# alvinwan/neural-backed-decision-trees

Measured on AMD Instinct MI355X. Metric: images/sec training SoftNBDT WRN28x10 CIFAR10, higher is better.
Workload: dtype bf16; 1 GPU; WideResNet-28-10 + SoftTreeSupLoss (induced-wrn28_10_cifar10, 10 leaves), CIFAR10-shaped 3x32x32, SGD m=0.9 wd=5e-4; batch_per_gpu=512, global_batch=512, parallelism=dp1

## Files before the change

include/nbdt_hip.h:

```cpp
#ifndef NBDT_HIP_H
#define NBDT_HIP_H

#include <stdint.h>

#ifdef __cplusplus
extern "C" {
#endif

#define NBDT_OK 0
#define NBDT_EINVAL (-1)
#define NBDT_EHIP (-2)
#define NBDT_ENOMEM (-3)

#define NBDT_F32 0
#define NBDT_BF16 1
#define NBDT_F16 2

const char* nbdt_last_error(void);
const char* nbdt_debug_last_igemm(void);
const char* nbdt_debug_last_igemm_full(void);
const char* nbdt_debug_last_wgrad(void);
int nbdt_version(void);
int nbdt_set_deterministic(int32_t on);
int nbdt_get_deterministic(void);
int nbdt_set_wgrad_store_epilogue(int32_t on);
int nbdt_get_wgrad_store_epilogue(void);
int nbdt_set_reserved_cus(int32_t n);
int nbdt_get_reserved_cus(void);
int nbdt_device_count(void);

int nbdt_weight_tile_batched(const void* src_bf16, const int64_t* table, int32_t n, int64_t total_tiles,
                             void* dst_bf16, void* stream);

typedef struct nbdt_tree nbdt_tree;
int nbdt_tree_create(int device, int num_classes, int num_inodes, int root,
                     const int32_t* node_off, const int32_t* slot_off, const int32_t* slot_cls,
                     const int32_t* cls_off, const int32_t* cls_slot, const int32_t* slot_next,
                     nbdt_tree** out);
int nbdt_tree_destroy(nbdt_tree* t);
int nbdt_tree_max_depth(const nbdt_tree* t);


int nbdt_soft_forward(const nbdt_tree* t, const void* z, int ztype, int64_t B, int64_t ldz,
                      float* P, void* stream);
int nbdt_soft_backward(const nbdt_tree* t, const void* z, int ztype, int64_t B, int64_t ldz,
                       const float* gP, float* gz, void* stream);
int nbdt_soft_tree_loss(const nbdt_tree* t, const void* z, int ztype, int64_t B, int64_t ldz,
                        const int64_t* y, float w_xent, float w_tree, float grad_scale,
                        float* row_loss, float* loss, float* gz, void* stream);
int nbdt_head_soft_tree_loss(const nbdt_tree* t, const float* pooled, const float* W, const float* bias, int64_t B,
                             int32_t K, const int64_t* y, float w_xent, float w_tree, float grad_scale,
                             float* row_loss, float* loss, float* z_out, float* gpooled, float* gW, float* gb,
                             void* stream);

int nbdt_hard_tree_loss(const nbdt_tree* t, const void* z, int ztype, int64_t B, int64_t ldz,
                        const int64_t* y, float w_xent, float w_node, float grad_scale,
                        float* row_loss, float* loss, float* gz, void* stream);
int nbdt_node_logits_backward(const nbdt_tree* t, const float* gs, int64_t B, float* gz, void* stream);
int nbdt_hard_forward(const nbdt_tree* t, const void* z, int ztype, int64_t B, int64_t ldz,
                      int64_t* pred, float* onehot, int32_t* path_node, int32_t* path_child,
                      float* path_prob, float* path_entropy, void* stream);
int nbdt_node_outputs(const nbdt_tree* t, const void* z, int ztype, int64_t B, int64_t ldz,
                      float* logits, float* probs, int64_t* preds, float* entropy, void* stream);

typedef struct nbdt_conv_desc {
  int32_t B, gh, gw;
  int32_t cin, cout;
  int32_t ntaps;
  int32_t tap_off[9];
  int32_t w_tap[9];
  int32_t w_ntaps;
  int32_t in_bs, in_hs, in_ws, in_base;
  int32_t out_bs, out_hs, out_ws, out_base;
  int32_t accumulate;
  int32_t wide_tile;
  int32_t ksplit;
  uint64_t w_tiled;
} nbdt_conv_desc;
int nbdt_conv_plan(const nbdt_conv_desc* d, int32_t* form, int32_t* ksplit);
int nbdt_conv_igemm(const nbdt_conv_desc* d, const void* in, const void* w, void* out,
                    const void* residual, void* stream);

int nbdt_conv_igemm_multi(const nbdt_conv_desc* descs, int32_t n, const void* in, const void* w, void* out,
                          void* stream);

typedef struct nbdt_conv_seg_slice {
  int32_t tensor;
  int32_t ch0;
  int32_t ntaps;
  int32_t tap[9];
  int32_t w_matrix;
  int32_t w_off[9];
} nbdt_conv_seg_slice;
typedef struct nbdt_conv_seg_class {
  int32_t nslices;
  const nbdt_conv_seg_slice* slices;
  int32_t out_bs, out_hs, out_ws, out_base;
} nbdt_conv_seg_class;
#define NBDT_SEG_MAX_SLICES 64
typedef struct nbdt_conv_seg_desc {
  int32_t B, gh, gw;
  int32_t cout;
  int32_t ntensors;
  int32_t pix_stride[4];
  int32_t nmatrices;
  int32_t w_row_stride[4];
  int32_t nclasses;
  nbdt_conv_seg_class cls[4];
  int32_t tile;
  int32_t nbuf;
} nbdt_conv_seg_desc;
int nbdt_conv_seg_create(const nbdt_conv_seg_desc* d, void** plan);
int nbdt_conv_seg_destroy(void* plan);
int nbdt_conv_seg_info(void* plan, int32_t* tile, int32_t* nbuf, int32_t* steps, int32_t* max_rounds,
                       int64_t* w_tile_elems);
int nbdt_conv_seg_tile_weights(void* plan, const void* const* w, void* w_tiles, void* stream);
int nbdt_conv_seg(void* plan, const void* const* in, const void* w_tiles, void* out, const void* residual,
                  float* bn_partials, void* stream);
int nbdt_conv_seg_steps(void* plan, int32_t cls, int32_t* out8, int32_t max_steps, int32_t* npro);

int nbdt_conv_igemm_stats(const nbdt_conv_desc* d, const void* in, const void* w, void* out,
                          const void* residual, float* bn_partials, void* stream);

int nbdt_conv_igemm_bnbwd(const nbdt_conv_desc* d, const void* in, const void* w, void* out,
                          const void* bn_x, const float* save_mean, const float* save_rstd,
                          const float* gamma, const float* beta, float* bn_partials, void* stream);
int nbdt_conv_igemm_affine(const nbdt_conv_desc* d, const void* in, const void* w, void* out,
                           const void* residual, const float* scale, const float* shift, int32_t act,
                           void* stream);

typedef struct nbdt_wgrad_desc {
  int32_t B, gh, gw;
  int32_t cin, cout;
  int32_t ntaps;
  int32_t tap_off[9];
  int32_t w_tap[9];
  int32_t w_ntaps;
  int32_t x_bs, x_hs, x_ws, x_base;
  int32_t g_bs, g_hs, g_ws, g_base;
  int32_t variant;
  int32_t cu_budget;
} nbdt_wgrad_desc;
int nbdt_conv_wgrad(const nbdt_wgrad_desc* d, const void* x, const void* gy, float* dw,
                    void* stream);
int nbdt_conv_wgrad_blocks(const nbdt_wgrad_desc* d);

int nbdt_weight_prep(const float* w, int32_t cout, int32_t taps, int32_t cin, void* w_bf16,
                     void* wd_bf16, void* stream);

int nbdt_weight_prep_batched(const float* flat, const int64_t* table, int32_t n_layers, int64_t total_tiles,
                             void* wd_flat, void* stream);

#define NBDT_BN_SLOTS 32
int nbdt_bn_stats(const void* x, int32_t B, int32_t H, int32_t W, int32_t C, float eps,
                  float momentum, float* running_mean, float* running_var, float* scratch,
                  float* save_mean, float* save_rstd, void* stream);
int nbdt_bn_finalize(int32_t B, int32_t H, int32_t W, int32_t C, float eps, float momentum,
                     float* running_mean, float* running_var, const float* bn_partials, float* save_mean,
                     float* save_rstd, void* stream);
int nbdt_bn_apply(const void* x, const float* save_mean, const float* save_rstd, const float* gamma,
                  const float* beta, const void* residual, int32_t relu, int32_t B, int32_t H,
                  int32_t W, int32_t C, void* y, void* stream);
int nbdt_bn_apply_s2d(const void* x, const float* save_mean, const float* save_rstd, const float* gamma,
                      const float* beta, int32_t relu, int32_t B, int32_t H, int32_t W, int32_t C, void* y,
                      void* stream);
int nbdt_bn_bwd_reduce(const void* gy, const void* y, const void* x, const float* save_mean,
                       const float* save_rstd, const float* gamma, const float* beta, int32_t relu,
                       int32_t B, int32_t H, int32_t W, int32_t C, float* scratch, float* dsum,
                       float* dgamma, float* dbeta, void* stream);
int nbdt_bn_bwd_fold(int32_t B, int32_t H, int32_t W, int32_t C, const float* bn_partials, float* dsum,
                     float* dgamma, float* dbeta, void* stream);
int nbdt_bn_bwd_apply(const void* gy, const void* y, const void* x, const float* save_mean,
                      const float* save_rstd, const float* gamma, const float* beta, const float* dsum,
                      const void* gx_add, int32_t relu, int32_t B, int32_t H, int32_t W, int32_t C,
                      void* gx, void* g_resid, void* stream);
int nbdt_bn_bwd_apply_cus(const void* gy, const void* x, const float* save_mean, const float* save_rstd,
                          const float* gamma, const float* beta, const float* dsum, const void* gx_add,
                          int32_t B, int32_t H, int32_t W, int32_t C, void* gx, int32_t cus, void* stream);
int nbdt_bn_bwd_reduce_cus(const void* gy, const void* x, const float* save_mean, const float* save_rstd,
                           const float* gamma, const float* beta, int32_t B, int32_t H, int32_t W, int32_t C,
                           float* scratch, float* dsum, float* dgamma, float* dbeta, int32_t cus, void* stream);
int nbdt_bn_bwd_cus(const void* gy, const void* x, const float* save_mean, const float* save_rstd, const float* gamma,
                    const float* beta, const void* gx_add, int32_t B, int32_t H, int32_t W, int32_t C, float* slots,
                    float* slots_other, float* dsum, float* dgamma, float* dbeta, void* gx, int32_t cus,
                    void* stream);
int nbdt_bn_relu_pool(const void* x, const float* save_mean, const float* save_rstd,
                      const float* gamma, const float* beta, int32_t B, int32_t H, int32_t W,
                      int32_t C, float* pooled, void* stream);
int nbdt_pool_bn_bwd_reduce(const float* gpooled, const void* x, const float* save_mean,
                            const float* save_rstd, const float* gamma, const float* beta,
                            int32_t B, int32_t H, int32_t W, int32_t C, float* scratch, float* dsum,
                            float* dgamma, float* dbeta, void* stream);
int nbdt_pool_bn_bwd_apply(const float* gpooled, const void* x, const float* save_mean,
                           const float* save_rstd, const float* gamma, const float* beta,
                           const float* dsum, int32_t B, int32_t H, int32_t W, int32_t C, void* gx,
                           void* stream);

#define NBDT_ACT_NONE 0
#define NBDT_ACT_RELU 1
#define NBDT_ACT_SWISH 2
int nbdt_bn_act_apply(const void* x, const float* save_mean, const float* save_rstd, const float* gamma,
                      const float* beta, int32_t act, const float* gate, const void* residual, int32_t B,
                      int32_t H, int32_t W, int32_t C, void* y, void* stream);
int nbdt_bn_act_pool(const void* x, const float* save_mean, const float* save_rstd, const float* gamma,
                     const float* beta, int32_t act, const void* mul, float scale, int32_t B, int32_t H,
                     int32_t W, int32_t C, float* out, void* stream);
int nbdt_bn_act_bwd(const void* gu, const float* gate, const float* gpool, const void* x,
                    const float* save_mean, const float* save_rstd, const float* gamma, const float* beta,
                    int32_t act, const void* gx_add, int32_t B, int32_t H, int32_t W, int32_t C,
                    float* scratch, float* dsum, float* dgamma, float* dbeta, void* gx, void* stream);
int nbdt_dwconv_fwd(const void* x, const float* w, int32_t B, int32_t H, int32_t W, int32_t C, int32_t k,
                    int32_t stride, void* y, float* bn_scratch , void* stream);
int nbdt_dwconv_bwd_data(const void* gy, const float* w, int32_t B, int32_t H, int32_t W, int32_t C,
                         int32_t k, int32_t stride, void* gx, void* stream);
int nbdt_dwconv_bwd_data_bn(const void* gy, const float* w, int32_t B, int32_t H, int32_t W, int32_t C, int32_t k,
                            void* gx, const void* bn_x, const float* save_mean, const float* save_rstd,
                            const float* gamma, const float* beta, float* scratch, void* stream);
int nbdt_bn_act_bwd_apply(const void* gu, const void* x, const float* save_mean, const float* save_rstd,
                          const float* gamma, const float* beta, int32_t act, const void* gx_add, int32_t B, int32_t H,
                          int32_t W, int32_t C, float* scratch, float* dsum, float* dgamma, float* dbeta, void* gx,
                          void* stream);
int nbdt_bn_act_se_sums(const void* gu, const void* x, const float* save_mean, const float* save_rstd,
                        const float* gamma, const float* beta, int32_t act, int32_t B, int32_t H, int32_t W, int32_t C,
                        float* sums, void* stream);
int nbdt_bn_act_se_bwd_apply(const void* gu, const float* gate, const float* gpool, float* sums, const void* x,
                             const float* save_mean, const float* save_rstd, const float* gamma, const float* beta,
                             int32_t act, int32_t B, int32_t H, int32_t W, int32_t C, float* dsum, float* dgamma,
                             float* dbeta, void* gx, void* stream);
int nbdt_dwconv_bwd_weight(const void* x, const void* gy, int32_t B, int32_t H, int32_t W, int32_t C,
                           int32_t k, int32_t stride, float* dw, void* stream);
int nbdt_se_gate_fwd(const float* pooled, const float* w1, const float* b1, const float* w2,
                     const float* b2, int32_t B, int32_t C, int32_t C_real, int32_t S, float* pre1,
                     float* gate, void* stream);
int nbdt_se_gate_bwd(const float* dgate, const float* gate, const float* pre1, const float* pooled,
                     const float* w1, const float* w2, int32_t B, int32_t C, int32_t C_real, int32_t S,
                     float* dpre2, float* dpre1, float* gpool, float* dw1, float* db1, float* dw2,
                     float* db2, void* stream);
int nbdt_se_param_grad(const float* dpre2, const float* dpre1, const float* pre1, const float* pooled,
                       int32_t B, int32_t C, int32_t C_real, int32_t S, float* dw1, float* db1, float* dw2,
                       float* db2, void* stream);
int nbdt_dropout_fwd(const float* x, int64_t n, float p, uint32_t seed, uint8_t* mask, float* y,
                     void* stream);
int nbdt_dropout_bwd(const float* gy, int64_t n, float p, const uint8_t* mask, float* gx, void* stream);

int nbdt_ref_conv(const nbdt_conv_desc* d, const float* in, const float* w, float* out, const float* residual,
                  void* stream);
int nbdt_ref_wgrad(const nbdt_wgrad_desc* d, const float* x, const float* gy, float* dw, void* stream);
int nbdt_ref_conv_seg(void* plan, const float* const* in, const float* const* w, float* out, const float* residual,
                      void* stream);
int nbdt_ref_bn_stats(const float* x, int32_t B, int32_t H, int32_t W, int32_t C, float eps, float momentum,
                      float* running_mean, float* running_var, float* save_mean, float* save_rstd, float* partials,
                      void* stream);
int nbdt_ref_bn_apply(const float* x, const float* save_mean, const float* save_rstd, const float* gamma,
                      const float* beta, const float* residual, int32_t relu, int32_t B, int32_t H, int32_t W,
                      int32_t C, float* y, void* stream);
int nbdt_ref_bn_apply_s2d(const float* x, const float* save_mean, const float* save_rstd, const float* gamma,
                          const float* beta, int32_t relu, int32_t B, int32_t H, int32_t W, int32_t C, float* y,
                          void* stream);
int nbdt_ref_bn_bwd(const float* gy, const float* gpooled, const float* y, const float* x, const float* save_mean,
                    const float* save_rstd, const float* gamma, const float* beta, int32_t relu, const float* gx_add,
                    int32_t B, int32_t H, int32_t W, int32_t C, int32_t reduce, float* dsum, float* dgamma,
                    float* dbeta, float* gx, float* g_resid, void* stream);
int nbdt_ref_bn_relu_pool(const float* x, const float* save_mean, const float* save_rstd, const float* gamma,
                          const float* beta, int32_t B, int32_t H, int32_t W, int32_t C, float* pooled, void* stream);
int nbdt_ref_stem_conv(const float* img, const float* w, int32_t B, int32_t H, int32_t W, int32_t cout_real,
                       int32_t cpad, int32_t stride, float* out, void* stream);
int nbdt_ref_stem_wgrad(const float* img, const float* gy, int32_t B, int32_t H, int32_t W, int32_t cout_real,
                        int32_t cpad, int32_t stride, float* dw, void* stream);
int nbdt_ref_bn_act_apply(const float* x, const float* save_mean, const float* save_rstd, const float* gamma,
                          const float* beta, int32_t act, const float* gate, const float* residual, int32_t B, int32_t H,
                          int32_t W, int32_t C, float* y, void* stream);
int nbdt_ref_bn_act_pool(const float* x, const float* save_mean, const float* save_rstd, const float* gamma,
                         const float* beta, int32_t act, const float* mul, float scale, int32_t B, int32_t H, int32_t W,
                         int32_t C, float* out, void* stream);
int nbdt_ref_bn_act_bwd(const float* gu, const float* gate, const float* gpool, const float* x, const float* save_mean,
                        const float* save_rstd, const float* gamma, const float* beta, int32_t act, const float* gx_add,
                        int32_t B, int32_t H, int32_t W, int32_t C, float* dsum, float* dgamma, float* dbeta, float* gx,
                        void* stream);
int nbdt_ref_dwconv_fwd(const float* x, const float* w, int32_t B, int32_t H, int32_t W, int32_t C, int32_t k,
                        int32_t stride, float* y, void* stream);
int nbdt_ref_dwconv_bwd_data(const float* gy, const float* w, int32_t B, int32_t H, int32_t W, int32_t C, int32_t k,
                             int32_t stride, float* gx, void* stream);
int nbdt_ref_dwconv_bwd_weight(const float* x, const float* gy, int32_t B, int32_t H, int32_t W, int32_t C, int32_t k,
                               int32_t stride, float* dw, void* stream);

int nbdt_stem_conv(const float* img, const float* w, int32_t B, int32_t H, int32_t W,
                   int32_t cout_real, int32_t cpad, int32_t stride, void* out, void* stream);
int nbdt_stem_wgrad(const float* img, const void* gy, int32_t B, int32_t H, int32_t W,
                    int32_t cout_real, int32_t cpad, int32_t stride, float* dw, void* stream);
int nbdt_linear_fwd(const float* x, const float* w, const float* b, int32_t B, int32_t K, int32_t N,
                    float* z, void* stream);
int nbdt_linear_bwd(const float* x, const float* w, const float* gz, int32_t B, int32_t K, int32_t N,
                    float* gx, float* gw, float* gb, void* stream);
int nbdt_sgd_step(float* p, float* g, float* buf, int64_t n, float lr, float momentum,
                  float weight_decay, float grad_scale, void* p_bf16, int32_t zero_grad, void* stream);

int nbdt_probe_mfma_stream(int32_t blocks, int32_t iters, float* sink, void* stream);
int nbdt_probe_lds_mfma(int32_t blocks, int32_t iters, int32_t variant, float* sink, void* stream);
// ... 6 lines not shown
```

neural-backed-decision-trees_amd/csrc/common.h:

```cpp
#pragma once
#include <hip/hip_runtime.h>
#include <hip/hip_bf16.h>
#include <hip/hip_fp16.h>
#include <stdint.h>
#include <stdio.h>
#include <string.h>

#include <mutex>

#include "../../include/nbdt_hip.h"

#if !defined(NBDT_TIMING_BUILD) &&                                                                                    \
    (defined(NBDT_WPP_NO_EPI) || defined(NBDT_WKS_NO_EXCHANGE) || defined(NBDT_WKS_DMA_IN_M) || defined(NBDT_WPP_MIN_STAGES) || defined(NBDT_WPP_FRAC8) || defined(NBDT_PP_KFRAC5) ||    \
     defined(NBDT_DMA_WTILED_FAKE) || defined(NBDT_PP_DUMMY_VALU) || defined(NBDT_PP_NO_PERSIST) || defined(NBDT_PP_NO_PAD) ||                    \
     defined(NBDT_HALO_NO_ACCUMULATE) || defined(NBDT_DW_TARGET) || defined(NBDT_DW_U) || defined(NBDT_HEAD_SPB) ||    \
     defined(NBDT_EPI_TIMING) || defined(NBDT_EPI_STATS_ATOMICS) || defined(NBDT_WGT_NSTAGE) || defined(NBDT_NO_XCD_CONTIGUOUS) || defined(NBDT_CUS_IN_FLIGHT) || defined(NBDT_NT_MIN_MB) || defined(NBDT_PLAIN_STORES) ||                      \
     (defined(NBDT_HEAD_SKIP) && (NBDT_HEAD_SKIP + 0) != 0) || (defined(NBDT_PP_ABLATE) && (NBDT_PP_ABLATE + 0) != 0) || \
     (defined(NBDT_PP_SCHED) && (NBDT_PP_SCHED + 0) != 0) || (defined(NBDT_PP_TIMING) && (NBDT_PP_TIMING + 0) != 0) ||  \
     (defined(NBDT_WPP_TIMING) && (NBDT_WPP_TIMING + 0) != 0) || (defined(NBDT_SEG_TIMING) && (NBDT_SEG_TIMING + 0) != 0) || (defined(NBDT_RULES_TIMING) && (NBDT_RULES_TIMING + 0) != 0))
#error "timing-experiment switch without -DNBDT_TIMING_BUILD: these switches change what the kernels compute (csrc/common.h)"
#endif
#ifdef NBDT_TIMING_BUILD
extern "C" __attribute__((weak, used, visibility("default"))) int nbdt_timing_build() { return 1; }
#endif

namespace nbdt {

extern thread_local char g_err[512];

inline int fail(int code, const char* fmt, const char* a = "", const char* b = "") {
  snprintf(g_err, sizeof(g_err), fmt, a, b);
  return code;
}

#define NBDT_HIP_CHECK(expr)                                                              \
  do {                                                                                    \
    hipError_t _e = (expr);                                                               \
    if (_e != hipSuccess) return nbdt::fail(NBDT_EHIP, "%s: %s", #expr, hipGetErrorString(_e)); \
  } while (0)

#define NBDT_REQUIRE(cond, msg)                                       \
  do {                                                                \
    if (!(cond)) return nbdt::fail(NBDT_EINVAL, "%s (%s)", msg, #cond); \
  } while (0)

#define NBDT_LAUNCH_CHECK() NBDT_HIP_CHECK(hipGetLastError())

struct DeviceAttr {
  static constexpr int kMaxDevices = 64;
  std::mutex m;
  size_t bytes[kMaxDevices] = {};
  int dev = 0;
  bool need(size_t want) {
    int d = 0;
    (void)hipGetDevice(&d);
    if (d < 0 || d >= kMaxDevices) d = kMaxDevices - 1;
    m.lock();
    dev = d;
    if (bytes[d] >= want && want > 0) { m.unlock(); return false; }
    return true;
  }
  void done(size_t want) { bytes[dev] = want ? want : 1; m.unlock(); }
  void abort() { m.unlock(); }
};
#define NBDT_ATTR_CHECK(site, expr)                                                       \
  do {                                                                                    \
    hipError_t _e = (expr);                                                               \
    if (_e != hipSuccess) { (site).abort(); return nbdt::fail(NBDT_EHIP, "%s: %s", #expr, hipGetErrorString(_e)); } \
  } while (0)

bool deterministic();
bool wgrad_store_epilogue();
int reserved_cus();
float* det_rows(hipStream_t st, size_t floats);
const char* det_rows_why();
int det_fold(hipStream_t st, const float* rows, int nrows, size_t n, float* dst);

typedef unsigned short bf16_t;

__device__ __forceinline__ float bf16_to_f32(bf16_t v) {
  return __uint_as_float(((unsigned)v) << 16);
}
__device__ __forceinline__ bf16_t f32_to_bf16(float f) {
  unsigned u = __float_as_uint(f);
  if ((u & 0x7fffffffu) > 0x7f800000u) return (bf16_t)((u >> 16) | 0x40);
  u += 0x7fffu + ((u >> 16) & 1u);
  return (bf16_t)(u >> 16);
}
__device__ __forceinline__ unsigned pack_bf16x2(float lo, float hi) {
  unsigned r;
  asm("v_cvt_pk_bf16_f32 %0, %1, %2" : "=v"(r) : "v"(lo), "v"(hi));
  return r;
}

struct FastDiv {
  unsigned mul, sh, d;
};
inline FastDiv make_fastdiv(unsigned d) {
  FastDiv f;
  f.d = d;
  if (d == 1) { f.mul = 0; f.sh = 0; return f; }
  unsigned s = 0;
  while ((1ull << s) < d) ++s;
  const unsigned long long num = 1ull << (31 + s);
  f.mul = (unsigned)((num + d - 1) / d);
  f.sh = s - 1;
  return f;
}
__device__ __forceinline__ unsigned fdiv(unsigned n, const FastDiv& f) {
  return f.d == 1 ? n : (__umulhi(n, f.mul) >> f.sh);
}

struct PadGeom {
  int B, H, W, C;
  int npix;
  int row;
  int img;
  FastDiv div_w, div_h;
};
inline PadGeom make_geom(int B, int H, int W, int C) {
  PadGeom g;
  g.B = B; g.H = H; g.W = W; g.C = C;
  g.npix = B * H * W;
  g.row = (W + 2) * C;
  g.img = (H + 2) * g.row;
  g.div_w = make_fastdiv((unsigned)W);
  g.div_h = make_fastdiv((unsigned)H);
  return g;
}
__device__ __forceinline__ int pad_offset(const PadGeom& g, int p) {
  const unsigned t = fdiv((unsigned)p, g.div_w);
  const int w = p - (int)t * g.W;
  const unsigned b = fdiv(t, g.div_h);
  const int h = (int)t - (int)b * g.H;
  return (int)b * g.img + (h + 1) * g.row + (w + 1) * g.C;
}

int wgrad_dma(const nbdt_wgrad_desc* d, const void* x, const void* gy, float* dw, hipStream_t st);

bool wgrad_taps_applicable(const nbdt_wgrad_desc* d);
int wgrad_taps(const nbdt_wgrad_desc* d, const void* x, const void* gy, float* dw, hipStream_t st);
int wgrad_taps_blocks(const nbdt_wgrad_desc* d);

bool wgrad_s2d_applicable(const nbdt_wgrad_desc* d);
int wgrad_s2d(const nbdt_wgrad_desc* d, const void* x, const void* gy, float* dw, hipStream_t st);
int wgrad_s2d_blocks(const nbdt_wgrad_desc* d);

struct BnBwdArgs {
  const void* x;
  const float *mean, *rstd, *gamma, *beta;
  const float *aff_scale = nullptr, *aff_shift = nullptr;
  int aff_act = 0;
};
int conv_igemm_dma(const nbdt_conv_desc* d, const void* in, const void* w, void* out, const void* res,
                   float* stats, const BnBwdArgs* bn, int M, hipStream_t st);
int conv_igemm_dma_multi(const nbdt_conv_desc* descs, int n, const void* in, const void* w, void* out, hipStream_t st);

struct HaloGeom {
  int ib, rb;
  int hw2;
  int himg;
  int hp;
  int a_instr;
  int a_bytes;
  int blocks_per_img;
  int nwv;
  int mw;
  int lpitch, limg;
  int pad, dv;
  int row_magic;
};
bool conv_halo_applicable(const nbdt_conv_desc* d, int M, HaloGeom* hg);
int conv_ksplit_rule(const nbdt_conv_desc& d, int nt, int items);
int conv_halo_items(const nbdt_conv_desc& d, const HaloGeom& hg, int M, int* nt_out);
extern thread_local const char* g_last_wgrad;
extern thread_local const char* g_last_igemm;
extern thread_local char g_last_igemm_full[128];
struct BnBwdArgs;
int conv3x3_halo(const nbdt_conv_desc* d, const HaloGeom& hg, const void* in, const void* w, void* out,
                 const void* res, float* stats, const BnBwdArgs* bn, int M, hipStream_t st);

}

__device__ __forceinline__ void glds16_s(const void* sbase, unsigned voff, unsigned lds_dst) {
  unsigned keep;
  asm volatile(
      "s_mov_b32 %0, m0\n\t"
      "s_mov_b32 m0, %3\n\t"
      "s_nop 2\n\t"
      "global_load_lds_dwordx4 %1, %2\n\t"
      "s_mov_b32 m0, %0"
      : "=&s"(keep)
      : "v"(voff), "s"(sbase), "s"(lds_dst)
      : "memory");
}

__device__ __forceinline__ void glds16_sf(const void* sbase, unsigned voff, unsigned lds_dst) {
  const unsigned long long b = (unsigned long long)sbase;
  const unsigned lo = __builtin_amdgcn_readfirstlane((unsigned)b), hi = __builtin_amdgcn_readfirstlane((unsigned)(b >> 32));
  glds16_s((const void*)(((unsigned long long)hi << 32) | lo), voff, __builtin_amdgcn_readfirstlane(lds_dst));
}

namespace nbdt {

typedef __attribute__((ext_vector_type(4))) unsigned u32x4_t;

template <bool NT>
__device__ __forceinline__ u32x4_t ld16_stream(const void* p) {
  if (NT) return __builtin_nontemporal_load((const u32x4_t*)p);
  return *(const u32x4_t*)p;
}
#ifndef NBDT_NT_MIN_MB
#define NBDT_NT_MIN_MB 96
#endif
inline bool stream_nt(long long tensor_bytes) { return tensor_bytes >= ((long long)NBDT_NT_MIN_MB << 20); }

template <bool WT = true>
__device__ __forceinline__ void st16(void* p, const u32x4_t v) {
#ifdef NBDT_PLAIN_STORES
  *(u32x4_t*)p = v;
#else
  if (WT) asm volatile("global_store_dwordx4 %0, %1, off sc1\n\ts_nop 2" ::"v"(p), "v"(v) : "memory");
  else *(u32x4_t*)p = v;
#endif
}

__device__ __forceinline__ void unpack8(const u32x4_t v, float* f) {
#pragma unroll
  for (int i = 0; i < 4; ++i) {
    f[2 * i] = __uint_as_float(v[i] << 16);
    f[2 * i + 1] = __uint_as_float(v[i] & 0xffff0000u);
  }
}
__device__ __forceinline__ u32x4_t pack8(const float* f) {
  u32x4_t v;
#pragma unroll
  for (int i = 0; i < 4; ++i) v[i] = pack_bf16x2(f[2 * i], f[2 * i + 1]);
  return v;
}

}
```

neural-backed-decision-trees_amd/csrc/rules.hip:

```cpp
#include "common.h"

#include <algorithm>
#include <vector>

namespace nbdt {
thread_local char g_err[512] = "";
}

using namespace nbdt;

struct nbdt_tree {
  int device;
  int C, N, R, L, root, max_depth;
  int sched_len;
  int32_t* d_all;
  const int32_t *node_off, *slot_off, *slot_cls, *cls_off, *cls_slot, *slot_next;
  const int32_t* sched;
};

struct TreeView {
  int C, N, R, L, root, max_depth, sched_len;
  int tl_ints;
  int staged;
  const int32_t *node_off, *slot_off, *slot_cls, *cls_off, *cls_slot, *slot_next, *sched;
// ... 823 lines not shown
  if (active)
    for (int c0 = g_tid; c0 < t.C; c0 += joint_of<TPS>() * TPS) {
      float d[joint_of<TPS>()];
      class_chains<TPS, ChainAdd>(t, o, c0, ds, stage, 0.f, d);
#pragma unroll
      for (int m = 0; m < joint_of<TPS>(); ++m)
        if (c0 + m * TPS < t.C) gz[sample * t.C + c0 + m * TPS] = gx[c0 + m * TPS] + d[m];
    }
}

__global__ __launch_bounds__(kBlock) void node_logits_bwd_kernel(TreeView t, const float* __restrict__ gs,
                                                                 int64_t B, float* __restrict__ gz) {
  const int64_t i = (int64_t)blockIdx.x * kBlock + threadIdx.x;
  if (i >= B * t.C) return;
  const int64_t b = i / t.C;
  const int c = (int)(i - b * t.C);
  gz[i] = class_grad_direct(t, c, gs + b * t.R);
}

__global__ __launch_bounds__(kBlock) void mean_kernel(const float* __restrict__ rows, int64_t n,
                                                      float* __restrict__ out) {
  __shared__ float red[kBlock / 64];
  float acc = 0.f;
  for (int64_t i = threadIdx.x; i < n; i += kBlock) acc += rows[i];
#pragma unroll
  for (int o = 32; o > 0; o >>= 1) acc += __shfl_xor(acc, o, 64);
  if ((threadIdx.x & 63) == 0) red[threadIdx.x >> 6] = acc;
  __syncthreads();
  if (threadIdx.x == 0) out[0] = (red[0] + red[1] + red[2] + red[3]) / (float)n;
}

template <int TPS, typename LD>
__global__ __launch_bounds__(block_of(TPS)) void hard_fwd_kernel(TreeView t, const void* z, int64_t B, int64_t ldz,
                                                          int64_t* __restrict__ pred,
                                                          float* __restrict__ onehot,
                                                          int32_t* __restrict__ path_node,
                                                          int32_t* __restrict__ path_child,
                                                          float* __restrict__ path_prob,
                                                          float* __restrict__ path_entropy) {
  extern __shared__ __attribute__((aligned(16))) float lds[];
  constexpr int SPB = block_of(TPS) / TPS;
  const int g = threadIdx.x / TPS, g_tid = threadIdx.x % TPS;
  const int64_t sample = (int64_t)blockIdx.x * SPB + g;
  const bool active = sample < B;
  const int stride = t.C + t.R + 8 + 2 * t.N + (t.staged ? t.L : 0);
  Gather<TPS> ga, gb;
  if (t.staged) ga.issue(t.slot_cls, t.L, active, g_tid);
  const TreeLds o = stage_tree<true>(t, lds);
  float* zs = lds + t.tl_ints + (size_t)g * stride;
  float* ss = zs + t.C;
  int* res = (int*)(ss + t.R);
  int* best_of = res + 8;
  int* next_of = best_of + t.N;
  float* stage = (float*)(next_of + t.N);
  load_and_node_logits<TPS, LD>(t, o, z, sample * ldz, active, g_tid, zs, ss, stage, ga, gb, nullptr);
  if (active)
    for (int n = g_tid; n < t.N; n += TPS) {
      const int b = o.node_off[n], e = o.node_off[n + 1];
      int best = b;
      for (int s = b + 1; s < e; ++s)
        if (ss[s] > ss[best]) best = s;
      best_of[n] = best;
      next_of[n] = o.slot_next[best];
    }
  __syncthreads();
  if (active && g_tid == 0) {
    int n = t.root, cls = -1;
    const bool want = path_node != nullptr;
    int d = 0;
    for (; d < t.max_depth; ++d) {
      const int best = best_of[n];
      if (want) {
        const int b = o.node_off[n], e = o.node_off[n + 1];
        const float m = ss[best];
        float sum = 0.f;
        for (int s = b; s < e; ++s) sum = sum + expf(ss[s] - m);
        const float eps = 1.1920928955078125e-07f;
        float tot = 0.f;
        for (int s = b; s < e; ++s) tot = tot + expf(ss[s] - m) / sum;
        float h = 0.f;
        for (int s = b; s < e; ++s) {
          const float p = (expf(ss[s] - m) / sum) / tot;
          h = h + p * logf(fminf(fmaxf(p, eps), 1.0f - eps));
        }
        const int64_t o = sample * t.max_depth + d;
        path_node[o] = n;
        path_child[o] = best - b;
        path_prob[o] = expf(ss[best] - m) / sum;
        path_entropy[o] = -h;
      }
      const int nx = next_of[n];
      if (nx >= 0) {
        n = nx;
      } else {
        cls = -nx - 1;
        ++d;
        break;
      }
    }
    if (want)
      for (; d < t.max_depth; ++d) {
        const int64_t o = sample * t.max_depth + d;
        path_node[o] = -1; path_child[o] = -1; path_prob[o] = 0.f; path_entropy[o] = 0.f;
      }
    pred[sample] = cls;
    res[0] = cls;
  }
  __syncthreads();
  if (active && onehot != nullptr) {
    const int cls = res[0];
    for (int c = g_tid; c < t.C; c += TPS) onehot[sample * t.C + c] = (c == cls) ? 1.f : 0.f;
  }
}

template <int TPS, typename LD>
__global__ __launch_bounds__(block_of(TPS)) void node_outputs_kernel(TreeView t, const void* z, int64_t B, int64_t ldz,
                                                              float* __restrict__ logits,
                                                              float* __restrict__ probs,
                                                              int64_t* __restrict__ preds,
                                                              float* __restrict__ entropy) {
  extern __shared__ __attribute__((aligned(16))) float lds[];
  constexpr int SPB = block_of(TPS) / TPS;
  const int g = threadIdx.x / TPS, g_tid = threadIdx.x % TPS;
  const int64_t sample = (int64_t)blockIdx.x * SPB + g;
  const bool active = sample < B;
  const int stride = t.C + 2 * t.R + (t.staged ? t.L : 0);
  Gather<TPS> ga, gb;
  if (t.staged) ga.issue(t.slot_cls, t.L, active, g_tid);
  const TreeLds o = stage_tree<false>(t, lds);
  float* zs = lds + t.tl_ints + (size_t)g * stride;
  float* ss = zs + t.C;
  float* ps = ss + t.R;
  load_and_node_logits<TPS, LD>(t, o, z, sample * ldz, active, g_tid, zs, ss, ps + t.R, ga, gb, nullptr);
  node_softmax<TPS>(t, o, active, g_tid, ss, ps);
  if (!active) return;
  for (int s = g_tid; s < t.R; s += TPS) {
    if (logits) logits[sample * t.R + s] = ss[s];
    if (probs) probs[sample * t.R + s] = ps[s];
  }
  for (int n = g_tid; n < t.N; n += TPS) {
    const int b = o.node_off[n], e = o.node_off[n + 1];
    if (preds) {
      int best = b;
      for (int s = b + 1; s < e; ++s)
        if (ss[s] > ss[best]) best = s;
      preds[sample * t.N + n] = best - b;
    }
    if (entropy) entropy[sample * t.N + n] = node_entropy(ps, b, e);
  }
}


extern "C" const char* nbdt_last_error(void) { return nbdt::g_err; }
extern "C" int nbdt_version(void) { return 108; }
extern "C" int nbdt_device_count(void) {
  int n = 0;
  if (hipGetDeviceCount(&n) != hipSuccess) return 0;
  return n;
}

static int pick_tps(int C, int R) { return (C <= 64 && R <= 64) ? 64 : (C <= 512 && R <= 512) ? 256 : 1024; }

static void build_slot_schedule(int R, const int32_t* slot_off, int lanes, std::vector<int32_t>* out, int* len) {
  std::vector<int> order(R);
  for (int s = 0; s < R; ++s) order[s] = s;
  auto length = [&](int s) { return slot_off[s + 1] - slot_off[s]; };
  std::stable_sort(order.begin(), order.end(), [&](int a, int b) { return length(a) > length(b); });
  const int waves = lanes / 64, chunks = (R + 63) / 64;
  std::vector<std::vector<int>> mine(waves);
  std::vector<long> load(waves, 0);
  for (int c = 0; c < chunks; ++c) {
    const int longest = length(order[c * 64]);
    int w = 0;
    for (int i = 1; i < waves; ++i)
      if (load[i] < load[w]) w = i;
    mine[w].push_back(c);
    load[w] += 64 + 8L * longest;
  }
  size_t rows = 0;
  for (auto& m : mine) rows = std::max(rows, m.size());
  const int n = (int)rows * lanes;
  out->assign((size_t)3 * n, -1);
  for (int w = 0; w < waves; ++w)
    for (size_t k = 0; k < mine[w].size(); ++k)
      for (int l = 0; l < 64; ++l) {
        const int i = mine[w][k] * 64 + l;
        if (i >= R) break;
        const int at = (int)k * lanes + w * 64 + l, s = order[i];
        (*out)[at] = s;
        (*out)[n + at] = slot_off[s];
        (*out)[2 * n + at] = slot_off[s + 1];
      }
  *len = n;
}

extern "C" int nbdt_tree_create(int device, int C, int N, int root, const int32_t* node_off,
                                const int32_t* slot_off, const int32_t* slot_cls, const int32_t* cls_off,
                                const int32_t* cls_slot, const int32_t* slot_next, nbdt_tree** out) {
  NBDT_REQUIRE(out && node_off && slot_off && slot_cls && cls_off && cls_slot && slot_next, "null argument");
  NBDT_REQUIRE(C > 0 && N > 0 && root >= 0 && root < N, "bad tree sizes");
  const int R = node_off[N];
  const int L = slot_off[R];
  NBDT_REQUIRE(R > 0 && L > 0 && cls_off[C] == L, "inconsistent CSR maps");
  for (int n = 0; n < N; ++n) NBDT_REQUIRE(node_off[n + 1] > node_off[n], "inner node without children");
  for (int s = 0; s < R; ++s) {
    NBDT_REQUIRE(slot_off[s + 1] > slot_off[s], "child without leaves");
    NBDT_REQUIRE(slot_next[s] < N && slot_next[s] >= -C, "bad slot_next");
  }
  for (int j = 0; j < L; ++j) {
    NBDT_REQUIRE(slot_cls[j] >= 0 && slot_cls[j] < C, "class index out of range");
    NBDT_REQUIRE(cls_slot[j] >= 0 && cls_slot[j] < R, "slot index out of range");
  }
  int max_depth = 0;
  {
    int* depth = new int[N];
    for (int n = 0; n < N; ++n) depth[n] = 1;
    bool changed = true;
    int iters = 0;
    while (changed && iters <= N + 1) {
      changed = false;
      ++iters;
      for (int n = 0; n < N; ++n)
        for (int s = node_off[n]; s < node_off[n + 1]; ++s)
          if (slot_next[s] >= 0 && depth[n] < depth[slot_next[s]] + 1) {
            depth[n] = depth[slot_next[s]] + 1;
            changed = true;
          }
    }
    max_depth = depth[root];
    delete[] depth;
    NBDT_REQUIRE(iters <= N + 1, "hierarchy has a cycle");
  }

  int prev = 0;
  NBDT_HIP_CHECK(hipGetDevice(&prev));
  NBDT_HIP_CHECK(hipSetDevice(device));
  std::vector<int32_t> sched;
  int sched_len = 0;
  build_slot_schedule(R, slot_off, pick_tps(C, R), &sched, &sched_len);
  nbdt_tree* t = new nbdt_tree();
  t->device = device; t->C = C; t->N = N; t->R = R; t->L = L; t->root = root; t->max_depth = max_depth;
  t->sched_len = sched_len;
  const size_t n_ints = (size_t)(N + 1) + (R + 1) + L + (C + 1) + L + R + sched.size();
  hipError_t e = hipMalloc((void**)&t->d_all, n_ints * sizeof(int32_t));
  if (e != hipSuccess) {
    delete t;
    (void)hipSetDevice(prev);
    return nbdt::fail(NBDT_ENOMEM, "hipMalloc(tree): %s", hipGetErrorString(e));
  }
  int32_t* host = new int32_t[n_ints];
  size_t o = 0;
  auto put = [&](const int32_t* src, size_t n, const int32_t** dst) {
    memcpy(host + o, src, n * sizeof(int32_t));
    *dst = t->d_all + o;
    o += n;
  };
  put(node_off, N + 1, &t->node_off);
  put(slot_off, R + 1, &t->slot_off);
  put(slot_cls, L, &t->slot_cls);
  put(cls_off, C + 1, &t->cls_off);
  put(cls_slot, L, &t->cls_slot);
  put(slot_next, R, &t->slot_next);
  put(sched.data(), sched.size(), &t->sched);
  e = hipMemcpy(t->d_all, host, n_ints * sizeof(int32_t), hipMemcpyHostToDevice);
  delete[] host;
  (void)hipSetDevice(prev);
  if (e != hipSuccess) {
    (void)hipFree(t->d_all);
    delete t;
    return nbdt::fail(NBDT_EHIP, "hipMemcpy(tree): %s", hipGetErrorString(e));
  }
  *out = t;
  return NBDT_OK;
}

extern "C" int nbdt_tree_destroy(nbdt_tree* t) {
  if (!t) return NBDT_OK;
  (void)hipFree(t->d_all);
  delete t;
  return NBDT_OK;
}

extern "C" int nbdt_tree_max_depth(const nbdt_tree* t) { return t ? t->max_depth : 0; }

static int pick_tps(const nbdt_tree* t) { return pick_tps(t->C, t->R); }

constexpr size_t kLdsBytes = 160 * 1024;
constexpr size_t kStagePad = 4;

template <typename... KA, typename... A>
static int launch_rules(void (*kernel)(KA...), unsigned grid, int block, size_t shmem, hipStream_t st,
                        A... args) {
  if (shmem > 64 * 1024)
    NBDT_HIP_CHECK(hipFuncSetAttribute(reinterpret_cast<const void*>(kernel),
                                       hipFuncAttributeMaxDynamicSharedMemorySize, (int)shmem));
  hipLaunchKernelGGL(kernel, dim3(grid), dim3(block), shmem, st, args...);
  NBDT_LAUNCH_CHECK();
  return NBDT_OK;
}

#define NBDT_DISPATCH_RULES(KERNEL, NEXT, BASE_FLOATS, ...)                                                \
  do {                                                                                               \
    const int tps = pick_tps(t);                                                                     \
    const int spb = block_of(tps) / tps;                                                             \
    size_t floats = (size_t)(BASE_FLOATS);                                                           \
    v.tl_ints = tree_lds_ints(t, NEXT);                                                              \
    v.staged = ((size_t)v.tl_ints + (size_t)spb * (floats + t->L) + kStagePad) * sizeof(float) <= kLdsBytes; \
// ... 193 lines not shown
```

neural-backed-decision-trees_amd/csrc/wgrad.hip:

```cpp
#include "common.h"

using namespace nbdt;

extern "C" int nbdt_conv_wgrad(const nbdt_wgrad_desc* d, const void* x, const void* gy, float* dw,
                               void* stream) {
  NBDT_REQUIRE(d && x && gy && dw, "null argument");
  NBDT_REQUIRE(d->cin > 0 && d->cin % 32 == 0 && d->cout > 0 && d->cout % 32 == 0, "channels must be multiples of 32");
  NBDT_REQUIRE(d->ntaps >= 1 && d->ntaps <= 9 && d->w_ntaps >= 1, "bad tap table");
  NBDT_REQUIRE(d->B > 0 && d->gh > 0 && d->gw > 0, "empty pixel grid");
  for (int t = 0; t < d->ntaps; ++t) {
    NBDT_REQUIRE(d->w_tap[t] >= 0 && d->w_tap[t] < d->w_ntaps, "bad w_tap");
    NBDT_REQUIRE(d->tap_off[t] % 8 == 0, "tap offsets must be 16-byte aligned");
  }
  NBDT_REQUIRE(d->x_bs % 8 == 0 && d->x_hs % 8 == 0 && d->x_ws % 8 == 0 && d->x_base % 8 == 0 &&
               d->g_bs % 8 == 0 && d->g_hs % 8 == 0 && d->g_ws % 8 == 0 && d->g_base % 8 == 0,
               "pixel offsets must be 16-byte aligned");
  NBDT_REQUIRE(d->cu_budget == 0 || (d->cu_budget >= 32 && d->cu_budget <= 256), "cu_budget must be 0 or 32..256");
  const int64_t M_all = (int64_t)d->B * d->gh * d->gw;
  NBDT_REQUIRE(M_all < (1ll << 31), "pixel grid too large");
  if (nbdt::wgrad_taps_applicable(d)) return nbdt::wgrad_taps(d, x, gy, dw, (hipStream_t)stream);
  if (d->variant != 3 && nbdt::wgrad_s2d_applicable(d)) return nbdt::wgrad_s2d(d, x, gy, dw, (hipStream_t)stream);
  NBDT_REQUIRE(d->variant == 0 || d->variant == 3, "variant 2 / 4 / 5 select between the dense 3x3 stride-1 kernels only");
  nbdt::g_last_wgrad = "conv_wgrad_dma_kernel";
  return nbdt::wgrad_dma(d, x, gy, dw, (hipStream_t)stream);
}

extern "C" int nbdt_conv_wgrad_blocks(const nbdt_wgrad_desc* d) {
  if (!d || d->cin <= 0 || d->cin % 32 != 0 || d->cout <= 0 || d->cout % 32 != 0 || d->ntaps != 9) return 0;
  if (d->B <= 0 || d->gh <= 0 || d->gw <= 0) return 0;
  if (d->cu_budget != 0 && (d->cu_budget < 32 || d->cu_budget > 256)) return 0;
  if (d->variant != 3 && nbdt::wgrad_s2d_applicable(d)) return nbdt::wgrad_s2d_blocks(d);
  return nbdt::wgrad_taps_blocks(d);
}

namespace nbdt { thread_local const char* g_last_wgrad = ""; }
extern "C" const char* nbdt_debug_last_wgrad(void) { return nbdt::g_last_wgrad; }
```

neural-backed-decision-trees_amd/csrc/wgrad_s2d.hip:

```cpp
#include "common.h"
#include <stdlib.h>
#include <algorithm>

using namespace nbdt;

typedef __attribute__((ext_vector_type(8))) short bf16x8;
typedef __attribute__((ext_vector_type(4))) short s16x4;
typedef __attribute__((ext_vector_type(4))) float f32x4;
typedef __attribute__((ext_vector_type(2))) unsigned u32x2;

namespace nbdt {
struct WgradS2dParams {
  nbdt_wgrad_desc d;
  const bf16_t* x;
  const bf16_t* gy;
  float* dw;
  long long dw_split_stride;
  int stages, stages_per_split, n_ci_blocks, splits, items, per_xcd;
  int store;
  int rs, cs;
  int x_slots, x_instr;
  int stages_per_row, rowgroups;
  int x_pix;
  FastDiv div_spr, div_rg;
};
}

template <int WM>
__global__ __launch_bounds__(512, 2) void conv_wgrad_s2d_kernel(nbdt::WgradS2dParams p) {
  constexpr int CG = 32 * WM;
  constexpr int KSP = 64;
  constexpr int PG = 2 * CG;
  constexpr int G_BYTES = KSP * PG;
  constexpr int G_INSTR = G_BYTES / 1024;
  constexpr int IPG = (G_INSTR + 7) / 8;
  constexpr int IPX = 3;
  constexpr int NSLOT = 4, PD = 3;
  extern __shared__ __attribute__((aligned(16))) unsigned char smem[];

  const nbdt_wgrad_desc& d = p.d;
  const int tid = threadIdx.x;
  const int lane = tid & 63;
  const int wave = __builtin_amdgcn_readfirstlane(tid >> 6);
  const int grp = wave >> 2, w4 = wave & 3;
  const int wm = w4 >> 1, wn = w4 & 1;

  const int item = (blockIdx.x & 7) * p.per_xcd + (blockIdx.x >> 3);
  if (item >= p.items) return;
  const int n_tiles = p.items / p.splits;
  const int tile = item % n_tiles;
  const int split = item / n_tiles;
  const int co_blk = tile / p.n_ci_blocks;
  const int ci_blk = tile - co_blk * p.n_ci_blocks;
  const int co0 = co_blk * CG;
  const int ci0 = ci_blk * 32;
  const int s_begin = split * p.stages_per_split;
  int s_end = s_begin + p.stages_per_split;
  s_end = s_end < p.stages ? s_end : p.stages;
  if (s_begin >= s_end) return;
  const int n_st = s_end - s_begin;

#define NBDT_PIN(x) __builtin_amdgcn_readfirstlane(x)
  const int g_bs = NBDT_PIN(d.g_bs), g_hs = NBDT_PIN(d.g_hs), g_ws = NBDT_PIN(d.g_ws);
  const int x_bs = NBDT_PIN(d.x_bs), x_hs = NBDT_PIN(d.x_hs), x_ws = NBDT_PIN(d.x_ws);
  const int rs = NBDT_PIN(p.rs), cs = NBDT_PIN(p.cs);
  const int x_instr = NBDT_PIN(p.x_instr), x_slots = NBDT_PIN(p.x_slots);
  const int x_bytes = x_instr * 1024;
  const int stage_bytes = G_BYTES + x_bytes;
  FastDiv dspr, drg;
  dspr.mul = NBDT_PIN(p.div_spr.mul); dspr.sh = NBDT_PIN(p.div_spr.sh); dspr.d = NBDT_PIN(p.div_spr.d);
  drg.mul = NBDT_PIN(p.div_rg.mul); drg.sh = NBDT_PIN(p.div_rg.sh); drg.d = NBDT_PIN(p.div_rg.d);
  const unsigned long long gy_u = (unsigned long long)p.gy, x_u = (unsigned long long)p.x;
  const bf16_t* gy_base = (const bf16_t*)(((unsigned long long)NBDT_PIN((unsigned)(gy_u >> 32)) << 32) |
                                          (unsigned)NBDT_PIN((unsigned)gy_u));
  const bf16_t* x_base = (const bf16_t*)(((unsigned long long)NBDT_PIN((unsigned)(x_u >> 32)) << 32) |
                                         (unsigned)NBDT_PIN((unsigned)x_u));
#undef NBDT_PIN
  const int C1 = cs + 1, R1 = rs + 1;
  const int off11 = 0, off10 = R1 * C1, off01 = off10 + R1 * cs, off00 = off01 + rs * C1;

  const unsigned lds_base = (unsigned)(size_t)(__attribute__((address_space(3))) unsigned char*)smem;
  unsigned g_voff[IPG];
#pragma unroll
  for (int k = 0; k < IPG; ++k) {
    const int pos = (wave + 8 * k) * 1024 + lane * 16;
    int px = pos / PG;
    const int j = (pos - px * PG) >> 4;
    const int src_chunk = j ^ (((px >> 3) & 1) << 1);
    px = px < KSP ? px : KSP - 1;
    g_voff[k] = (unsigned)((px / cs) * g_hs + (px % cs) * g_ws + d.g_base + co0 + src_chunk * 8) * 2u;
  }
  unsigned x_voff[IPX];
#pragma unroll
  for (int k = 0; k < IPX; ++k) {
    int slot = 16 * (wave + 8 * k) + (lane >> 2);
    slot = slot < x_slots ? slot : x_slots - 1;
    int pp, qq, rel;
    if (slot < off10) { pp = 1; qq = 1; rel = slot - off11; }
    else if (slot < off01) { pp = 1; qq = 0; rel = slot - off10; }
    else if (slot < off00) { pp = 0; qq = 1; rel = slot - off01; }
    else { pp = 0; qq = 0; rel = slot - off00; }
    const int cq = cs + qq;
    const int i = rel / cq, j = rel - i * cq;
    const int src_chunk = (lane & 3) ^ ((((j >> 3) ^ i) & 1) << 1);
    x_voff[k] = (unsigned)((i - pp + 1) * x_hs + (j - qq + 1) * x_ws + (2 * pp + qq) * d.cin + ci0 + src_chunk * 8) * 2u;
  }
  int n_mine = 0;
#pragma unroll
  for (int k = 0; k < IPX; ++k) n_mine += (wave + 8 * k < x_instr) ? 1 : 0;
#pragma unroll
  for (int k = 0; k < IPG; ++k) n_mine += (wave + 8 * k < G_INSTR) ? 1 : 0;

  auto stage_off = [&](int stage, int& g_stage, int& x_stage) {
    const unsigned st = (unsigned)stage;
    const unsigned q1m = __umulhi(st, dspr.mul) >> dspr.sh;
    const unsigned q1 = dspr.d == 1 ? st : q1m;
    const int sc = (int)(st - q1 * dspr.d);
    const unsigned bm = __umulhi(q1, drg.mul) >> drg.sh;
    const unsigned b = drg.d == 1 ? q1 : bm;
    const int rg = (int)(q1 - b * drg.d);
    const int r0 = rg * rs, c0 = sc * cs;
    g_stage = (int)b * g_bs + r0 * g_hs + c0 * g_ws;
    x_stage = (int)b * x_bs + r0 * x_hs + c0 * x_ws;
  };
  auto issue = [&](int slot_i, int g_stage, int x_stage) {
    const unsigned dst0 = lds_base + slot_i * stage_bytes;
#pragma unroll
    for (int k = 0; k < IPG; ++k)
      if (wave + 8 * k < G_INSTR) glds16_s(gy_base + g_stage, g_voff[k], dst0 + (wave + 8 * k) * 1024);
#pragma unroll
    for (int k = 0; k < IPX; ++k)
      if (wave + 8 * k < x_instr) glds16_s(x_base + x_stage, x_voff[k], dst0 + G_BYTES + (wave + 8 * k) * 1024);
  };

  f32x4 acc[9][WM];
#pragma unroll
  for (int t = 0; t < 9; ++t)
#pragma unroll
    for (int a = 0; a < WM; ++a) acc[t][a] = f32x4{0.f, 0.f, 0.f, 0.f};

  typedef const __attribute__((address_space(3))) unsigned char* lds_cptr;
  typedef __attribute__((address_space(3))) s16x4* lds_tr;
  const lds_cptr smem3 = (lds_cptr)smem;
  const int g4 = lane >> 4, t16 = lane & 15;
  const int pr = t16 >> 2;
  const int c8 = (t16 & 3) * 8;
  int g_lane_off[2];
#pragma unroll
  for (int a = 0; a < 2; ++a)
    g_lane_off[a] = (grp * 32 + 8 * g4 + pr) * PG + (((wm * WM + a) ^ (g4 & 1)) * 32) + c8;
  int xrel1[3], xrel1c[3], xrel0[3];
  {
    const int k = grp * 32 + 8 * g4;
    const int row_l = k / cs, col_l = k - row_l * cs;
#pragma unroll
    for (int r = 0; r < 3; ++r) {
      const int pp = r != 1 ? 1 : 0;
      const int i = row_l + (r == 2 ? 1 : 0);
      const int sub1 = pp ? off11 : off01, sub0 = pp ? off10 : off00;
      const int j = col_l + pr, jc = j + 8;
      xrel1[r] = G_BYTES + c8 + (((sub1 + i * C1 + j) << 6) | (((((j >> 3) ^ i) ^ wn) & 1) << 5));
      xrel1c[r] = G_BYTES + c8 + (((sub1 + i * C1 + jc) << 6) | (((((jc >> 3) ^ i) ^ wn) & 1) << 5));
      xrel0[r] = G_BYTES + c8 + (((sub0 + i * cs + j) << 6) | (((((j >> 3) ^ i) ^ wn) & 1) << 5));
    }
  }

#pragma unroll
  for (int u = 0; u < PD; ++u)
    if (u < n_st) {
      int gs, xs;
      stage_off(s_begin + u, gs, xs);
      issue(u, gs, xs);
    }
  asm volatile("s_waitcnt vmcnt(0)" ::: "memory");
  __builtin_amdgcn_s_barrier();
  if (grp == 1) __builtin_amdgcn_s_barrier();
  __builtin_amdgcn_sched_barrier(0);

  lds_cptr xa1[3], xa1c[3], xa0[3];
  lds_cptr ga[2];
  ga[0] = smem3 + g_lane_off[0];
  ga[1] = smem3 + g_lane_off[1];
#pragma unroll
  for (int r = 0; r < 3; ++r) {
    xa1[r] = smem3 + xrel1[r];
    xa1c[r] = smem3 + xrel1c[r];
    xa0[r] = smem3 + xrel0[r];
  }
  auto advance = [&](int from_slot, int to_slot) {
    int delta = (to_slot - from_slot) * stage_bytes;
    asm volatile("" : "+s"(delta));
    ga[0] += delta;
    ga[1] += delta;
#pragma unroll
    for (int r = 0; r < 3; ++r) { xa1[r] += delta; xa1c[r] += delta; xa0[r] += delta; }
  };
  int slot_c = 0, slot_n = 1 % NSLOT, slot_d = PD % NSLOT;
  int g_next = 0, x_next = 0;
  if (PD < n_st) stage_off(s_begin + PD, g_next, x_next);

  for (int u = 0; u < n_st; ++u) {
    bf16x8 gf[WM];
// ... 9 lines not shown
    for (int r = 0; r < 3; ++r) {
      xw1[r][0] = __builtin_bit_cast(u32x2, __builtin_amdgcn_ds_read_tr16_b64_v4i16((lds_tr)xa1[r]));
      xw1[r][1] = __builtin_bit_cast(u32x2, __builtin_amdgcn_ds_read_tr16_b64_v4i16((lds_tr)(xa1[r] + 256)));
      xw1[r][2] = __builtin_bit_cast(u32x2, __builtin_amdgcn_ds_read_tr16_b64_v4i16((lds_tr)xa1c[r]));
      xw0[r][0] = __builtin_bit_cast(u32x2, __builtin_amdgcn_ds_read_tr16_b64_v4i16((lds_tr)xa0[r]));
      xw0[r][1] = __builtin_bit_cast(u32x2, __builtin_amdgcn_ds_read_tr16_b64_v4i16((lds_tr)(xa0[r] + 256)));
    }
    if (u + PD <= n_st) {
      switch (n_mine) {
#define NBDT_CASE(K) case K: asm volatile("s_waitcnt vmcnt(%0)" ::"n"(K) : "memory"); break;
        NBDT_CASE(1) NBDT_CASE(2) NBDT_CASE(3) NBDT_CASE(4) NBDT_CASE(5) NBDT_CASE(6)
#undef NBDT_CASE
        default: asm volatile("s_waitcnt vmcnt(0)" ::: "memory"); break;
      }
    } else {
      asm volatile("s_waitcnt vmcnt(0)" ::: "memory");
    }
    if (u + PD < n_st) issue(slot_d, g_next, x_next);
    asm volatile("s_waitcnt lgkmcnt(0)" ::: "memory");
    __builtin_amdgcn_sched_barrier(0);
    __builtin_amdgcn_s_barrier();
    __builtin_amdgcn_sched_barrier(0);
    __builtin_amdgcn_s_setprio(1);
    advance(slot_c, slot_n);
    stage_off(s_begin + u + 1 + PD, g_next, x_next);
#pragma unroll
    for (int t = 0; t < 9; ++t) {
      const int r = t / 3, sft = t % 3;
      u32x4_t v;
      if (sft == 1) {
        v = u32x4_t{xw0[r][0][0], xw0[r][0][1], xw0[r][1][0], xw0[r][1][1]};
      } else {
        const u32x2 A = xw1[r][0], B = xw1[r][1], C = xw1[r][2];
        if (sft == 0) v = u32x4_t{A[0], A[1], B[0], B[1]};
        else v = u32x4_t{__builtin_amdgcn_alignbit(A[1], A[0], 16), __builtin_amdgcn_alignbit(B[0], A[1], 16),
                         __builtin_amdgcn_alignbit(B[1], B[0], 16), __builtin_amdgcn_alignbit(C[0], B[1], 16)};
      }
      const bf16x8 xf = __builtin_bit_cast(bf16x8, v);
#pragma unroll
      for (int a = 0; a < WM; ++a)
        acc[t][a] = __builtin_amdgcn_mfma_f32_16x16x32_bf16(gf[a], xf, acc[t][a], 0, 0, 0);
    }
#pragma unroll
    for (int i = 0; i < 9 * WM; ++i) {
      __builtin_amdgcn_sched_group_barrier(0x008, 1, 0);
      __builtin_amdgcn_sched_group_barrier(0x002, 1, 0);
      __builtin_amdgcn_sched_group_barrier(0x004, 1, 0);
    }
#pragma unroll
    for (int r = 0; r < 3; ++r) asm volatile("" : "+v"(xa1[r]), "+v"(xa1c[r]), "+v"(xa0[r]));
    asm volatile("" : "+v"(ga[0]), "+v"(ga[1]));
    __builtin_amdgcn_s_setprio(0);
    __builtin_amdgcn_sched_barrier(0);
    __builtin_amdgcn_s_barrier();
    __builtin_amdgcn_sched_barrier(0);
    slot_c = slot_n;
    slot_n = slot_n + 1 == NSLOT ? 0 : slot_n + 1;
    slot_d = slot_d + 1 == NSLOT ? 0 : slot_d + 1;
  }
  if (grp == 0) __builtin_amdgcn_s_barrier();
  __builtin_amdgcn_sched_barrier(0);
  {
    typedef __attribute__((address_space(3))) f32x4* lds_f4;
    const lds_f4 ex = (lds_f4)(__attribute__((address_space(3))) unsigned char*)smem + (w4 * (5 * WM) * 64 + lane);
    if (grp == 1) {
#pragma unroll
      for (int t = 0; t < 5; ++t)
#pragma unroll
        for (int a = 0; a < WM; ++a) ex[(t * WM + a) * 64] = acc[t][a];
    }
    __syncthreads();
    if (grp == 0) {
#pragma unroll
      for (int t = 0; t < 5; ++t)
#pragma unroll
        for (int a = 0; a < WM; ++a) acc[t][a] += ex[(t * WM + a) * 64];
    }
    __syncthreads();
    if (grp == 0) {
#pragma unroll
      for (int t = 5; t < 9; ++t)
#pragma unroll
        for (int a = 0; a < WM; ++a) ex[((t - 5) * WM + a) * 64] = acc[t][a];
    }
    __syncthreads();
    if (grp == 1) {
#pragma unroll
      for (int t = 5; t < 9; ++t)
#pragma unroll
        for (int a = 0; a < WM; ++a) acc[t][a] += ex[((t - 5) * WM + a) * 64];
    }
  }
  const int ci = ci0 + wn * 16 + t16;
#pragma unroll
  for (int t = 0; t < 9; ++t) {
    if ((t < 5) != (grp == 0)) continue;
    const int w_tap = d.w_tap[t];
#pragma unroll
    for (int a = 0; a < WM; ++a)
#pragma unroll
      for (int r = 0; r < 4; ++r) {
        const int co = co0 + (wm * WM + a) * 16 + 4 * g4 + r;
        float* const dst = p.dw + (int64_t)split * p.dw_split_stride + ((int64_t)co * d.w_ntaps + w_tap) * d.cin + ci;
        if (p.store) *dst = acc[t][a][r];
        else atomicAdd(dst, acc[t][a][r]);
      }
  }
}

namespace nbdt {

static int s2d_wm(int cout) {
  const int mt = cout / 32;
  return mt % 5 == 0 ? 5 : (mt % 4 == 0 ? 4 : (mt % 2 == 0 ? 2 : 1));
}

static bool s2d_geometry(const nbdt_wgrad_desc* d, WgradS2dParams* p) {
  const int gw = d->gw, gh = d->gh, ks = 64;
  if (gw % 8 != 0 || !(gw % ks == 0 || ks % gw == 0)) return false;
  int rs = gw >= ks ? 1 : ks / gw;
  int cs = gw >= ks ? ks : gw;
  if (gw >= 64) { if (gw % 32 != 0 || gh % 2 != 0) return false; rs = 2; cs = 32; }
  if (gh % rs != 0) return false;
  const int slots = (2 * rs + 1) * (2 * cs + 1);
  const int x_instr = (slots + 15) / 16;
  if (x_instr > 24) return false;
  const size_t stage = (size_t)64 * 64 * s2d_wm(d->cout) + (size_t)x_instr * 1024;
  if (4 * stage > 160 * 1024) return false;
  if (!p) return true;
  p->rs = rs; p->cs = cs;
  p->x_slots = slots; p->x_instr = x_instr;
  p->stages = (int)((long long)d->B * gh * gw / ks);
  p->stages_per_row = gw / cs;
  p->rowgroups = gh / rs;
  p->div_spr = make_fastdiv((unsigned)p->stages_per_row);
  p->div_rg = make_fastdiv((unsigned)p->rowgroups);
  return true;
}

bool wgrad_s2d_applicable(const nbdt_wgrad_desc* d) {
  if (d->ntaps != 9 || d->w_ntaps != 9 || d->x_base != 0) return false;
  if (d->x_ws != 4 * d->cin || d->x_hs != (d->gw + 2) * d->x_ws || d->x_bs != (d->gh + 2) * d->x_hs) return false;
  if (d->g_ws != d->cout || d->g_hs != (d->gw + 2) * d->cout) return false;
  for (int t = 0; t < 9; ++t) {
    const int r = t / 3, s = t % 3;
    if (d->w_tap[t] != t) return false;
    if (d->tap_off[t] != (r != 0) * d->x_hs + (s != 0) * d->x_ws + (2 * (r != 1) + (s != 1)) * d->cin) return false;
  }
  if ((long long)d->B * d->x_bs * 2 >= (1ll << 32) || (long long)d->B * d->g_bs * 2 >= (1ll << 32)) return false;
  if ((long long)d->B * d->gh * d->gw < 64 * 64) return false;
  return s2d_geometry(d, nullptr);
}

static void s2d_split(WgradS2dParams& p, int wm) {
  const nbdt_wgrad_desc& d = p.d;
  p.n_ci_blocks = d.cin / 32;
  const int tiles = (d.cout / (32 * wm)) * p.n_ci_blocks;
  int cus = d.cu_budget > 0 ? d.cu_budget : 256;
  cus = std::max(8, std::min(cus, 256 - reserved_cus()));
  int splits = cus / tiles;
  const int max_splits = p.stages / 16 > 0 ? p.stages / 16 : 1;
  if (splits > max_splits) splits = max_splits;
  if (splits < 1) splits = 1;
  p.stages_per_split = (p.stages + splits - 1) / splits;
  splits = (p.stages + p.stages_per_split - 1) / p.stages_per_split;
  p.splits = splits;
  p.items = tiles * splits;
  p.per_xcd = (p.items + 7) / 8;
}

int wgrad_s2d_blocks(const nbdt_wgrad_desc* d) {
  WgradS2dParams p;
  p.d = *d;
  if (!s2d_geometry(d, &p)) return 0;
  s2d_split(p, s2d_wm(d->cout));
  return p.per_xcd * 8 < p.items ? p.per_xcd * 8 : p.items;
}

template <int WM>
static int launch_s2d(WgradS2dParams& p, hipStream_t st) {
  const nbdt_wgrad_desc& d = p.d;
  s2d_split(p, WM);
  const size_t shmem = (size_t)4 * (64 * 64 * WM + (size_t)p.x_instr * 1024);
  const void* fn = reinterpret_cast<const void*>(&conv_wgrad_s2d_kernel<WM>);
  static DeviceAttr site;
  if (site.need(shmem)) {
    NBDT_ATTR_CHECK(site, hipFuncSetAttribute(fn, hipFuncAttributeMaxDynamicSharedMemorySize, (int)shmem));
    site.done(shmem);
  }
  float* const dw = p.dw;
  const size_t dw_elems = (size_t)d.cout * d.w_ntaps * d.cin;
  p.dw_split_stride = 0;
  p.store = ((wgrad_store_epilogue() && p.splits <= 64 && d.cu_budget == 0) || deterministic()) ? 1 : 0;
  if (p.store) {
    float* rows = det_rows(st, (size_t)p.splits * dw_elems);
    if (!rows && !deterministic()) {
      p.store = 0;
    } else {
      if (!rows) return nbdt::fail(NBDT_ENOMEM, "weight gradient: %s (%s)", "no workspace for the per-split gradients",
                                   nbdt::det_rows_why());
      p.dw = rows;
      p.dw_split_stride = (long long)dw_elems;
    }
  }
  void* args[] = {(void*)&p};
  NBDT_HIP_CHECK(hipLaunchKernel(fn, dim3(p.per_xcd * 8), dim3(512), args, shmem, st));
  g_last_wgrad = "conv_wgrad_s2d_kernel";
  if (p.dw != dw) return det_fold(st, p.dw, p.splits, dw_elems, dw);
  return NBDT_OK;
}

int wgrad_s2d(const nbdt_wgrad_desc* d, const void* x, const void* gy, float* dw, hipStream_t st) {
  WgradS2dParams p;
  p.d = *d;
  p.x = (const bf16_t*)x;
  p.gy = (const bf16_t*)gy;
  p.dw = dw;
  p.x_pix = 4 * d->cin;
  if (!s2d_geometry(d, &p)) return nbdt::fail(NBDT_EINVAL, "%s%s", "space-to-depth weight gradient: shape does not fit", "");
  const int wm = s2d_wm(d->cout);
  if (wm == 5) return launch_s2d<5>(p, st);
  if (wm == 4) return launch_s2d<4>(p, st);
  if (wm == 2) return launch_s2d<2>(p, st);
  return launch_s2d<1>(p, st);
}

}
```

neural-backed-decision-trees_amd/nbdt/_C.py:

```python
import ctypes
import os
from ctypes import POINTER, c_char_p, c_float, c_int, c_int32, c_int64, c_void_p

import numpy as np
import torch

_LIBPATH = os.environ.get("NBDT_HIP_LIB") or os.path.join(os.path.dirname(os.path.abspath(__file__)), "_lib",
                                                         "libnbdt_hip.so")
_lib = None

NBDT_F32, NBDT_BF16, NBDT_F16 = 0, 1, 2
_ZTYPE = {torch.float32: NBDT_F32, torch.bfloat16: NBDT_BF16, torch.float16: NBDT_F16}


class NBDTHipError(RuntimeError):
    pass


class ConvDesc(ctypes.Structure):
    _fields_ = [
        ("B", c_int32), ("gh", c_int32), ("gw", c_int32),
        ("cin", c_int32), ("cout", c_int32),
        ("ntaps", c_int32),
        ("tap_off", c_int32 * 9), ("w_tap", c_int32 * 9), ("w_ntaps", c_int32),
        ("in_bs", c_int32), ("in_hs", c_int32), ("in_ws", c_int32), ("in_base", c_int32),
        ("out_bs", c_int32), ("out_hs", c_int32), ("out_ws", c_int32), ("out_base", c_int32),
        ("accumulate", c_int32),
        ("wide_tile", c_int32),
        ("ksplit", c_int32),
        ("w_tiled", ctypes.c_uint64),
    ]


class WgradDesc(ctypes.Structure):
    _fields_ = [
        ("B", c_int32), ("gh", c_int32), ("gw", c_int32),
        ("cin", c_int32), ("cout", c_int32),
        ("ntaps", c_int32),
        ("tap_off", c_int32 * 9), ("w_tap", c_int32 * 9), ("w_ntaps", c_int32),
        ("x_bs", c_int32), ("x_hs", c_int32), ("x_ws", c_int32), ("x_base", c_int32),
        ("g_bs", c_int32), ("g_hs", c_int32), ("g_ws", c_int32), ("g_base", c_int32),
        ("variant", c_int32),
        ("cu_budget", c_int32),
    ]


class ConvSegSlice(ctypes.Structure):
    _fields_ = [("tensor", c_int32), ("ch0", c_int32), ("ntaps", c_int32), ("tap", c_int32 * 9),
                ("w_matrix", c_int32), ("w_off", c_int32 * 9)]


class ConvSegClass(ctypes.Structure):
    _fields_ = [("nslices", c_int32), ("slices", POINTER(ConvSegSlice)),
                ("out_bs", c_int32), ("out_hs", c_int32), ("out_ws", c_int32), ("out_base", c_int32)]


class ConvSegDesc(ctypes.Structure):
    _fields_ = [("B", c_int32), ("gh", c_int32), ("gw", c_int32), ("cout", c_int32),
                ("ntensors", c_int32), ("pix_stride", c_int32 * 4),
                ("nmatrices", c_int32), ("w_row_stride", c_int32 * 4),
                ("nclasses", c_int32), ("cls", ConvSegClass * 4),
                ("tile", c_int32), ("nbuf", c_int32)]


_P = c_void_p
_I32P = POINTER(c_int32)

SIGNATURES = {
    "nbdt_last_error": (c_char_p, []),
    "nbdt_version": (c_int, []),
    "nbdt_device_count": (c_int, []),
    "nbdt_set_deterministic": (c_int, [c_int32]),
    "nbdt_get_deterministic": (c_int, []),
    "nbdt_set_wgrad_store_epilogue": (c_int, [c_int32]),
    "nbdt_get_wgrad_store_epilogue": (c_int, []),
    "nbdt_set_reserved_cus": (c_int, [c_int32]),
    "nbdt_probe_mfma_stream": (c_int, [c_int32, c_int32, _P, _P]),
    "nbdt_probe_lds_mfma": (c_int, [c_int32, c_int32, c_int32, _P, _P]),
    "nbdt_get_reserved_cus": (c_int, []),
    "nbdt_tree_create": (c_int, [c_int, c_int, c_int, c_int, _I32P, _I32P, _I32P, _I32P, _I32P, _I32P,
                                 POINTER(c_void_p)]),
    "nbdt_tree_destroy": (c_int, [c_void_p]),
    "nbdt_tree_max_depth": (c_int, [c_void_p]),
    "nbdt_debug_last_igemm": (c_char_p, []),
    "nbdt_debug_last_igemm_full": (c_char_p, []),
    "nbdt_debug_last_wgrad": (c_char_p, []),
    "nbdt_conv_wgrad_blocks": (c_int, [_P]),
    "nbdt_conv_plan": (c_int, [_P, _P, _P]),
    "nbdt_soft_forward": (c_int, [c_void_p, _P, c_int, c_int64, c_int64, _P, _P]),
    "nbdt_soft_backward": (c_int, [c_void_p, _P, c_int, c_int64, c_int64, _P, _P, _P]),
    "nbdt_soft_tree_loss": (c_int, [c_void_p, _P, c_int, c_int64, c_int64, _P, c_float, c_float, c_float,
                                    _P, _P, _P, _P]),
    "nbdt_head_soft_tree_loss": (c_int, [c_void_p, _P, _P, _P, c_int64, c_int32, _P, c_float, c_float, c_float,
                                         _P, _P, _P, _P, _P, _P, _P]),
    "nbdt_hard_tree_loss": (c_int, [c_void_p, _P, c_int, c_int64, c_int64, _P, c_float, c_float, c_float,
                                    _P, _P, _P, _P]),
    "nbdt_node_logits_backward": (c_int, [c_void_p, _P, c_int64, _P, _P]),
    "nbdt_hard_forward": (c_int, [c_void_p, _P, c_int, c_int64, c_int64, _P, _P, _P, _P, _P, _P, _P]),
    "nbdt_node_outputs": (c_int, [c_void_p, _P, c_int, c_int64, c_int64, _P, _P, _P, _P, _P]),
    "nbdt_conv_igemm": (c_int, [POINTER(ConvDesc), _P, _P, _P, _P, _P]),
    "nbdt_conv_igemm_multi": (c_int, [_P, c_int32, _P, _P, _P, _P]),
    "nbdt_conv_igemm_stats": (c_int, [POINTER(ConvDesc), _P, _P, _P, _P, _P, _P]),
    "nbdt_conv_seg_create": (c_int, [POINTER(ConvSegDesc), POINTER(c_void_p)]),
    "nbdt_conv_seg_destroy": (c_int, [c_void_p]),
    "nbdt_conv_seg_info": (c_int, [c_void_p, _I32P, _I32P, _I32P, _I32P, POINTER(c_int64)]),
    "nbdt_conv_seg_steps": (c_int, [c_void_p, c_int32, _I32P, c_int32, _I32P]),
    "nbdt_conv_seg_tile_weights": (c_int, [c_void_p, POINTER(c_void_p), _P, _P]),
    "nbdt_conv_seg": (c_int, [c_void_p, POINTER(c_void_p), _P, _P, _P, _P, _P]),
    "nbdt_ref_conv_seg": (c_int, [c_void_p, POINTER(c_void_p), POINTER(c_void_p), _P, _P, _P]),
    "nbdt_bn_apply_s2d": (c_int, [_P, _P, _P, _P, _P, c_int32, c_int32, c_int32, c_int32, c_int32, _P, _P]),
    "nbdt_ref_bn_apply_s2d": (c_int, [_P, _P, _P, _P, _P, c_int32, c_int32, c_int32, c_int32, c_int32, _P, _P]),
    "nbdt_bn_finalize": (c_int, [c_int32, c_int32, c_int32, c_int32, c_float, c_float, _P, _P, _P, _P, _P, _P]),
    "nbdt_conv_igemm_bnbwd": (c_int, [POINTER(ConvDesc), _P, _P, _P, _P, _P, _P, _P, _P, _P, _P]),
    "nbdt_conv_igemm_affine": (c_int, [POINTER(ConvDesc), _P, _P, _P, _P, _P, _P, c_int32, _P]),
    "nbdt_bn_bwd_fold": (c_int, [c_int32, c_int32, c_int32, c_int32, _P, _P, _P, _P, _P]),
    "nbdt_bn_bwd_apply_cus": (c_int, [_P, _P, _P, _P, _P, _P, _P, _P, c_int32, c_int32, c_int32, c_int32, _P, c_int32, _P]),
    "nbdt_bn_bwd_reduce_cus": (c_int, [_P, _P, _P, _P, _P, _P, c_int32, c_int32, c_int32, c_int32, _P, _P, _P, _P, c_int32, _P]),
    "nbdt_bn_bwd_cus": (c_int, [_P, _P, _P, _P, _P, _P, _P, c_int32, c_int32, c_int32, c_int32, _P, _P, _P, _P, _P, _P,
                                c_int32, _P]),
    "nbdt_conv_wgrad": (c_int, [POINTER(WgradDesc), _P, _P, _P, _P]),
    "nbdt_ref_conv": (c_int, [POINTER(ConvDesc), _P, _P, _P, _P, _P]),
    "nbdt_ref_wgrad": (c_int, [POINTER(WgradDesc), _P, _P, _P, _P]),
    "nbdt_ref_bn_stats": (c_int, [_P, c_int32, c_int32, c_int32, c_int32, c_float, c_float, _P, _P, _P, _P, _P, _P]),
    "nbdt_ref_bn_apply": (c_int, [_P, _P, _P, _P, _P, _P, c_int32, c_int32, c_int32, c_int32, c_int32, _P, _P]),
    "nbdt_ref_bn_bwd": (c_int, [_P, _P, _P, _P, _P, _P, _P, _P, c_int32, _P, c_int32, c_int32, c_int32, c_int32,
                                c_int32, _P, _P, _P, _P, _P, _P]),
    "nbdt_ref_bn_relu_pool": (c_int, [_P, _P, _P, _P, _P, c_int32, c_int32, c_int32, c_int32, _P, _P]),
    "nbdt_ref_stem_conv": (c_int, [_P, _P, c_int32, c_int32, c_int32, c_int32, c_int32, c_int32, _P, _P]),
    "nbdt_ref_stem_wgrad": (c_int, [_P, _P, c_int32, c_int32, c_int32, c_int32, c_int32, c_int32, _P, _P]),
    "nbdt_ref_bn_act_apply": (c_int, [_P, _P, _P, _P, _P, c_int32, _P, _P, c_int32, c_int32, c_int32, c_int32, _P, _P]),
    "nbdt_ref_bn_act_pool": (c_int, [_P, _P, _P, _P, _P, c_int32, _P, c_float, c_int32, c_int32, c_int32, c_int32, _P,
                                     _P]),
    "nbdt_ref_bn_act_bwd": (c_int, [_P, _P, _P, _P, _P, _P, _P, _P, c_int32, _P, c_int32, c_int32, c_int32, c_int32, _P,
                                    _P, _P, _P, _P]),
    "nbdt_ref_dwconv_fwd": (c_int, [_P, _P, c_int32, c_int32, c_int32, c_int32, c_int32, c_int32, _P, _P]),
    "nbdt_ref_dwconv_bwd_data": (c_int, [_P, _P, c_int32, c_int32, c_int32, c_int32, c_int32, c_int32, _P, _P]),
    "nbdt_ref_dwconv_bwd_weight": (c_int, [_P, _P, c_int32, c_int32, c_int32, c_int32, c_int32, c_int32, _P, _P]),
    "nbdt_weight_prep": (c_int, [_P, c_int32, c_int32, c_int32, _P, _P, _P]),
    "nbdt_weight_prep_batched": (c_int, [_P, _P, c_int32, c_int64, _P, _P]),
    "nbdt_weight_tile_batched": (c_int, [_P, _P, c_int32, c_int64, _P, _P]),
    "nbdt_bn_stats": (c_int, [_P, c_int32, c_int32, c_int32, c_int32, c_float, c_float, _P, _P, _P, _P, _P, _P]),
    "nbdt_bn_apply": (c_int, [_P, _P, _P, _P, _P, _P, c_int32, c_int32, c_int32, c_int32, c_int32, _P, _P]),
    "nbdt_bn_bwd_reduce": (c_int, [_P, _P, _P, _P, _P, _P, _P, c_int32, c_int32, c_int32, c_int32, c_int32,
                                   _P, _P, _P, _P, _P]),
    "nbdt_bn_bwd_apply": (c_int, [_P, _P, _P, _P, _P, _P, _P, _P, _P, c_int32, c_int32, c_int32, c_int32,
                                  c_int32, _P, _P, _P]),
    "nbdt_bn_relu_pool": (c_int, [_P, _P, _P, _P, _P, c_int32, c_int32, c_int32, c_int32, _P, _P]),
    "nbdt_pool_bn_bwd_reduce": (c_int, [_P, _P, _P, _P, _P, _P, c_int32, c_int32, c_int32, c_int32, _P, _P,
                                        _P, _P, _P]),
    "nbdt_pool_bn_bwd_apply": (c_int, [_P, _P, _P, _P, _P, _P, _P, c_int32, c_int32, c_int32, c_int32, _P,
                                       _P]),
    "nbdt_stem_conv": (c_int, [_P, _P, c_int32, c_int32, c_int32, c_int32, c_int32, c_int32, _P, _P]),
    "nbdt_stem_wgrad": (c_int, [_P, _P, c_int32, c_int32, c_int32, c_int32, c_int32, c_int32, _P, _P]),
    "nbdt_bn_act_apply": (c_int, [_P, _P, _P, _P, _P, c_int32, _P, _P, c_int32, c_int32, c_int32, c_int32, _P, _P]),
    "nbdt_bn_act_pool": (c_int, [_P, _P, _P, _P, _P, c_int32, _P, c_float, c_int32, c_int32, c_int32, c_int32,
                                 _P, _P]),
    "nbdt_bn_act_bwd": (c_int, [_P, _P, _P, _P, _P, _P, _P, _P, c_int32, _P, c_int32, c_int32, c_int32, c_int32,
                                _P, _P, _P, _P, _P, _P]),
    "nbdt_dwconv_fwd": (c_int, [_P, _P, c_int32, c_int32, c_int32, c_int32, c_int32, c_int32, _P, _P, _P]),
    "nbdt_dwconv_bwd_data": (c_int, [_P, _P, c_int32, c_int32, c_int32, c_int32, c_int32, c_int32, _P, _P]),
    "nbdt_dwconv_bwd_data_bn": (c_int, [_P, _P, c_int32, c_int32, c_int32, c_int32, c_int32, _P, _P, _P, _P, _P, _P, _P, _P]),
    "nbdt_bn_act_bwd_apply": (c_int, [_P, _P, _P, _P, _P, _P, c_int32, _P, c_int32, c_int32, c_int32, c_int32,
                                      _P, _P, _P, _P, _P, _P]),
    "nbdt_bn_act_se_sums": (c_int, [_P, _P, _P, _P, _P, _P, c_int32, c_int32, c_int32, c_int32, c_int32, _P, _P]),
    "nbdt_bn_act_se_bwd_apply": (c_int, [_P, _P, _P, _P, _P, _P, _P, _P, _P, c_int32, c_int32, c_int32, c_int32, c_int32,
                                         _P, _P, _P, _P, _P]),
    "nbdt_dwconv_bwd_weight": (c_int, [_P, _P, c_int32, c_int32, c_int32, c_int32, c_int32, c_int32, _P, _P]),
    "nbdt_se_gate_fwd": (c_int, [_P, _P, _P, _P, _P, c_int32, c_int32, c_int32, c_int32, _P, _P, _P]),
    "nbdt_se_gate_bwd": (c_int, [_P, _P, _P, _P, _P, _P, c_int32, c_int32, c_int32, c_int32, _P, _P, _P, _P, _P,
                                 _P, _P, _P]),
    "nbdt_se_param_grad": (c_int, [_P, _P, _P, _P, c_int32, c_int32, c_int32, c_int32, _P, _P, _P, _P, _P]),
    "nbdt_dropout_fwd": (c_int, [_P, c_int64, c_float, ctypes.c_uint32, _P, _P, _P]),
    "nbdt_dropout_bwd": (c_int, [_P, c_int64, c_float, _P, _P, _P]),
    "nbdt_linear_fwd": (c_int, [_P, _P, _P, c_int32, c_int32, c_int32, _P, _P]),
    "nbdt_linear_bwd": (c_int, [_P, _P, _P, c_int32, c_int32, c_int32, _P, _P, _P, _P]),
    "nbdt_sgd_step": (c_int, [_P, _P, _P, c_int64, c_float, c_float, c_float, c_float, _P, c_int32, _P]),
}


def _missing(name):
    def raiser(*_a, **_k):
        raise NBDTHipError(f"{_LIBPATH} does not export {name}: stale build, re-run build()")
    return raiser


def exported_symbols():
    l = ctypes.CDLL(_LIBPATH)
    return [n for n in SIGNATURES if hasattr(l, n)]


def lib():
    global _lib
    if _lib is None:
        if not os.path.exists(_LIBPATH):
            raise NBDTHipError(
                f"{_LIBPATH} is missing: build it with `python __graft_entry__.py build` "
                "(hipcc --offload-arch=gfx950).  There is no CPU fallback for the NBDT hot path.")
        l = ctypes.CDLL(_LIBPATH)
        if hasattr(l, "nbdt_timing_build") and os.environ.get("NBDT_ALLOW_TIMING_BUILD") != "1":
            raise NBDTHipError(f"{_LIBPATH} is a timing-experiment build (exports nbdt_timing_build): its kernels skip "
                               "work on purpose.  Set NBDT_ALLOW_TIMING_BUILD=1 in a measurement script; never train with it.")
        for name, (res, args) in SIGNATURES.items():
            try:
                fn = getattr(l, name)
            except AttributeError:
                setattr(l, name, _missing(name))
                continue
            fn.restype = res
            fn.argtypes = args
        _lib = l
    return _lib


def libpath():
    return _LIBPATH


def check(rc):
    if rc != 0:
        raise NBDTHipError(f"libnbdt_hip error {rc}: {lib().nbdt_last_error().decode()}")


def ptr(t):
    return None if t is None else c_void_p(t.data_ptr())


_raw_stream = getattr(torch._C, "_cuda_getCurrentRawStream", lambda idx: torch.cuda.current_stream(idx).cuda_stream)


def stream_of(t):
    return c_void_p(_raw_stream(t.device.index))


def require_gpu(t, what):
    if not t.is_cuda:
        raise NBDTHipError(
            f"{what}: tensor is on {t.device}; the NBDT hot path runs on MI355X only "
            "(no CPU fallback -- move inputs to a HIP device)")


def ztype_of(t):
    try:
        return _ZTYPE[t.dtype]
    except KeyError:
        raise NBDTHipError(f"unsupported logits dtype {t.dtype}") from None


class TreeHandle:

    def __init__(self, flat, device_index):
        self.flat = flat
        self.device_index = device_index
        out = c_void_p()
        as_p = lambda a: a.ctypes.data_as(_I32P)
        check(lib().nbdt_tree_create(
            int(device_index), flat.num_classes, flat.num_inodes, flat.root,
            as_p(flat.node_off), as_p(flat.slot_off), as_p(flat.slot_cls),
            as_p(flat.cls_off), as_p(flat.cls_slot), as_p(flat.slot_next), ctypes.byref(out)))
        self.h = out
        self.max_depth = lib().nbdt_tree_max_depth(self.h)

    def __del__(self):
        try:
            if getattr(self, "h", None) and _lib is not None:
                _lib.nbdt_tree_destroy(self.h)
        except Exception:
            pass


def _rows(z, handle):
    if z.dim() != 2:
        raise NBDTHipError(f"rules layer expects [B, C] logits, got shape {tuple(z.shape)}")
    if z.shape[1] != handle.flat.num_classes:
# ... 129 lines not shown
```

neural-backed-decision-trees_amd/nbdt/engine.py:

```python
import math

import torch

from nbdt import _C, ops

SIDE_STREAM_PRIORITY = 0

ALIGN = 8

_SIDE_STREAMS = {}


def side_stream(device):
    dev = torch.device(device)
    key = (dev.type, dev.index if dev.index is not None else torch.cuda.current_device())
    if key not in _SIDE_STREAMS:
        _SIDE_STREAMS[key] = torch.cuda.Stream(device=dev, priority=SIDE_STREAM_PRIORITY)
    return _SIDE_STREAMS[key]


def _pad32(c):
    return (c + 31) // 32 * 32


# ... 16 lines not shown
        self.n += (numel + ALIGN - 1) // ALIGN * ALIGN

    def finalize(self):
        n = (self.n + 3) // 4 * 4
        host = torch.zeros(n, dtype=torch.float32)
        for name, init in self.inits:
            off, shape = self.entries[name]
            numel = math.prod(shape)
            init(host[off:off + numel].view(shape))
        self.flat = host.to(self.device)
        self.grad = torch.zeros_like(self.flat)
        self.mom = torch.zeros_like(self.flat)
        self.bf16 = self.flat.to(torch.bfloat16)

    def _view(self, buf, name):
        off, shape = self.entries[name]
        return buf[off:off + math.prod(shape)].view(shape)

    def _cached(self, which, buf, name):
        cache = self.__dict__.setdefault("_views", {})
        hit = cache.get((which, name))
        if hit is not None and hit[1] is buf:
            return hit[0]
        v = self._view(buf, name)
        cache[(which, name)] = (v, buf)
        return v

    def p(self, name):
        return self._cached(0, self.flat, name)

    def g(self, name):
        return self._cached(1, self.grad, name)

    def pb(self, name):
        return self._cached(2, self.bf16, name)

    def refresh_bf16(self):
        self.bf16.copy_(self.flat)

    def zero_grad(self):
        self.grad.zero_()


class Conv:

    def __init__(self, store, name, cin_real, cout_real, k, stride, gen, init="kaiming_a0"):
        self.store, self.name = store, name
        self.cin_real, self.cout_real, self.k, self.stride = cin_real, cout_real, k, stride
        self.cin, self.cout = _pad32(cin_real), _pad32(cout_real)
        self.taps = k * k
        fan_in = cin_real * k * k
        if init == "kaiming_a0":
            bound = math.sqrt(2.0) * math.sqrt(3.0 / fan_in)
        else:
            bound = 1.0 / math.sqrt(fan_in)

        def init(v):
            v.zero_()
            v[:cout_real, :, :cin_real].uniform_(-bound, bound, generator=gen)

        store.add(name, (self.cout, self.taps, self.cin), init)
        self._plans = {}
        self.wd = None
        self.merge_parity_classes = True

    def logical(self, buf):
        v = self.store._view(buf, self.name).view(self.cout, self.k, self.k, self.cin)
        return v[:self.cout_real, :, :, :self.cin_real].permute(0, 3, 1, 2)

    def plan(self, B, Hi, Wi):
        key = (B, Hi, Wi)
        if key not in self._plans:
            self._plans[key] = self._make_plan(B, Hi, Wi)
        return self._plans[key]

    def _make_plan(self, B, Hi, Wi):
        p = self._raw_plan(B, Hi, Wi)
        if getattr(self, "wt_fwd", None) is not None:
            p[0].w_tiled = self.wt_fwd.data_ptr()
            for descs in (p[1], p[2]):
                if descs is not None and len(descs) == 1:
                    descs[0].w_tiled = self.wt_dgrad.data_ptr()
        return p

    def _raw_plan(self, B, Hi, Wi):
        args = (B, Hi, Wi, self.cin, self.cout, self.k, self.stride)
        plain_dgrad = None if (self.k == 1 and self.stride == 2) else ops.conv_dgrad_descs(*args, accumulate=False)
        plan = (ops.conv_fwd_desc(*args), plain_dgrad, ops.conv_dgrad_descs(*args, accumulate=True),
                ops.conv_wgrad_desc(*args))
        for d in (plan[0], plan[3]):
            d.flop_channels = (self.cin_real, self.cout_real)
        for descs in (plan[1], plan[2]):
            for d in descs or ():
                d.flop_channels = (self.cout_real, self.cin_real)
        return plan

    def numel(self):
        return self.cout * self.taps * self.cin

    def _w_for(self, x):
        return self.store.p(self.name) if x.dtype == torch.float32 else self.store.pb(self.name)

    def _wd_for(self, g):
        return self.wd32 if g.dtype == torch.float32 else self.wd

    def forward(self, x, out, residual=None, bn_scratch=None):
        B, Hp, Wp, _ = x.shape
        ops.conv_igemm(self.plan(B, Hp - 2, Wp - 2)[0], x, self._w_for(x), out, residual, bn_scratch)

    def forward_affine(self, x, out, bn, act=1, residual=None):
        B, Hp, Wp, _ = x.shape
        scale, shift = bn.eval_affine()
        ops.conv_igemm_affine(self.plan(B, Hp - 2, Wp - 2)[0], x, self.store.pb(self.name), out, scale, shift, act,
                              residual)

    def backward_data(self, gout, gin, accumulate=False, bn=None, bn_x=None, partials=None):
        B, Hp, Wp, _ = gin.shape
        plan = self.plan(B, Hp - 2, Wp - 2)
        descs = plan[2] if accumulate else plan[1]
        if bn is not None:
            assert len(descs) == 1 and not accumulate
            ops.conv_igemm_bnbwd(descs[0], gout, self.wd, gin, bn_x, bn.mean, bn.rstd, bn.gamma, bn.beta, partials)
            return
        if len(descs) > 1 and self.merge_parity_classes:
            ops.conv_igemm_multi(descs, gout, self._wd_for(gout), gin)
            return
        for d in descs:
            ops.conv_igemm(d, gout, self._wd_for(gout), gin)

    def s2d_plan(self, B, Hi, Wi):
        key = ("s2d", B, Hi, Wi)
        if key not in self._plans:
            fwd = ops.conv_fwd_desc_s2d_1x1(B, Hi, Wi, self.cin, self.cout) if self.k == 1 else None
            wg = ops.conv_wgrad_desc_s2d(B, Hi, Wi, self.cin, self.cout, self.k)
            for d in (fwd, wg):
                if d is not None:
                    d.flop_channels = (self.cin_real, self.cout_real)
            self._plans[key] = (fwd, wg)
        return self._plans[key]

    def forward_s2d(self, xs, out, Hi, Wi):
        ops.conv_igemm(self.s2d_plan(xs.shape[0], Hi, Wi)[0], xs, self._w_for(xs), out)

    def backward_weight_s2d(self, xs, gout, Hi, Wi, cu_budget=0):
        desc = self.s2d_plan(xs.shape[0], Hi, Wi)[1]
        side = getattr(self, "side_stream", None)
        if side is None:
            ops.conv_wgrad(desc, xs, gout, self.store.g(self.name), cu_budget)
            return
        main = torch.cuda.current_stream(xs.device)
        side.wait_stream(main)
        with torch.cuda.stream(side):
            ops.conv_wgrad(desc, xs, gout, self.store.g(self.name), cu_budget)

    def backward_weight(self, x, gout, cu_budget=0):
        B, Hp, Wp, _ = x.shape
        side = getattr(self, "side_stream", None)
        if side is None:
            ops.conv_wgrad(self.plan(B, Hp - 2, Wp - 2)[3], x, gout, self.store.g(self.name), cu_budget)
            return
        main = torch.cuda.current_stream(x.device)
        side.wait_stream(main)
        with torch.cuda.stream(side):
            ops.conv_wgrad(self.plan(B, Hp - 2, Wp - 2)[3], x, gout, self.store.g(self.name), cu_budget)


class SegOp:

    def __init__(self, plan, sources, sources32, on_side):
        self.plan, self.sources, self.sources32, self.on_side = plan, sources, sources32, on_side
        self.tiles = None

    def retile(self):
        self.tiles = self.plan.tile_weights(self.sources(), out=self.tiles)

    def __call__(self, ins, out, bn_scratch=None):
        if ins[0].dtype == torch.float32:
            self.plan(ins, self.sources32(), out, bn_scratch=bn_scratch)
        else:
            self.plan(ins, self.tiles, out, bn_scratch=bn_scratch)


class BatchNorm:
    def __init__(self, store, name, c_real, scratch_owner):
        self.store, self.name, self.c_real = store, name, c_real
        self.C = _pad32(c_real)
        store.add(name + ".weight", (self.C,), lambda v: v.fill_(1.0))
        store.add(name + ".bias", (self.C,), lambda v: v.zero_())
        dev = store.device
        self.running_mean = torch.zeros(self.C, device=dev)
        self.running_var = torch.ones(self.C, device=dev)
        self.num_batches_tracked = 0
        self.mean = torch.empty(self.C, device=dev)
        self.rstd = torch.empty(self.C, device=dev)
        self.dsum = torch.empty(2 * self.C, device=dev)
        self.owner = scratch_owner
        self._affine = None

    def eval_affine(self):
        if self._affine is None:
            scale = self.gamma * torch.rsqrt(self.running_var + ops.BN_EPS)
            self._affine = (scale.contiguous(), (self.beta - self.running_mean * scale).contiguous())
        return self._affine

    @property
    def gamma(self):
        return self.store.p(self.name + ".weight")

    @property
    def beta(self):
        return self.store.p(self.name + ".bias")

    def stats(self, x, training, fused=False):
        if training:
            self._affine = None
            if fused:
                ops.bn_finalize(x, self.owner.partials(x), self.mean, self.rstd, self.running_mean,
                                self.running_var)
            else:
                ops.bn_stats(x, self.owner.scratch(self.C), self.mean, self.rstd, self.running_mean,
                             self.running_var)
            self.num_batches_tracked += 1
        else:
            self.mean.copy_(self.running_mean)
            torch.rsqrt(self.running_var + ops.BN_EPS, out=self.rstd)

    def apply(self, x, y, relu=True, residual=None):
        ops.bn_apply(x, self.mean, self.rstd, self.gamma, self.beta, y, relu=relu, residual=residual)

    def backward_fused(self, gy, x, gx, partials, gx_add=None, cus=0):
        ops.bn_bwd_fused(gy, x, self.mean, self.rstd, self.gamma, self.beta, partials, self.dsum,
                         self.store.g(self.name + ".weight"), self.store.g(self.name + ".bias"), gx, gx_add=gx_add,
                         cus=cus)

    def backward_cus(self, gy, x, gx, cus, gx_add=None):
        scratch = self.owner.slot_pair(self.C) if self.owner.fuse_bn_fold else self.owner.scratch(self.C)
        ops.bn_bwd_cus(gy, x, self.mean, self.rstd, self.gamma, self.beta, scratch, self.dsum,
                       self.store.g(self.name + ".weight"), self.store.g(self.name + ".bias"), gx, cus, gx_add=gx_add)

    def backward(self, gy, y, x, gx, relu=True, gx_add=None, g_resid=None):
        ops.bn_bwd(gy, y, x, self.mean, self.rstd, self.gamma, self.owner.scratch(self.C), self.dsum,
                   self.store.g(self.name + ".weight"), self.store.g(self.name + ".bias"), gx, relu=relu,
                   gx_add=gx_add, g_resid=g_resid, beta=self.beta)


class _Engine:

    def __init__(self, device, seed):
        self.device = torch.device(device)
        if self.device.type != "cuda":
            raise RuntimeError("the NBDT backbone engine runs on MI355X only (no CPU fallback)")
        self.store = ParamStore(self.device)
        self.gen = torch.Generator().manual_seed(seed)
        self._scratch = None
        self._bufs = {}
        self.convs, self.bns = [], []
        self.training = True
        self.act_dtype = torch.bfloat16
        self.debug_keep = False
        self.debug_share_serial = False
        self.debug_join_each_unit = False
        self.fuse_stats = True
        self.fuse_eval = True
        self.share_bn2_tensors, self.share_bn1_tensors = 5, 6
        self.fuse_bn_fold = True
        self.fuse_dw_bn_bwd = True
        self.fuse_bn1_bwd = True
        self._side = None
        self._cu_share = None
        self._share_join = False
        self._share_split = (False, 250.0)
        self._share_calibrated = True
        self.cu_share_report = None
        self._overlap = True
        self.use_seg = True
        self._seg_ops = {}
        self.seg_share = True
        self.seg_join = None
        self.share_fused_hw = 0
        self.share_stage_us = {}
        self.share_scale_batch = True
        self.share_fused_target_us = 200.0

    def seg_op(self, key, build, sources, sources32, on_side=False):
        op = self._seg_ops.get(key)
        if op is None:
            op = SegOp(build(), sources, sources32, on_side)
            if self.act_dtype != torch.float32:
                if on_side and self._side is not None and self._overlap:
                    self._side.wait_stream(torch.cuda.current_stream(self.device))
                    with torch.cuda.stream(self._side):
                        op.retile()
                    torch.cuda.current_stream(self.device).wait_stream(self._side)
                else:
                    op.retile()
            self._seg_ops[key] = op
        return op

    def _retile_seg(self, on_side):
        if self.act_dtype == torch.float32:
            return
        for op in self._seg_ops.values():
            if op.on_side == on_side:
                op.retile()

    def s2d_buf(self, key, B, H, W, C):
        k = (key, "s2d", B, H, W, C)
        if k not in self._bufs:
            self._bufs[k] = ops.s2d_buffer(B, H, W, C, self.device, self.act_dtype)
        return self._bufs[k]

    def scratch(self, C):
        need = ops.BN_SLOTS * 2 * C
        if self._scratch is None or self._scratch.numel() < need:
            self._scratch = torch.zeros(max(need, ops.BN_SLOTS * 2 * 2048), device=self.device)
        return self._scratch

    def slot_pair(self, C):
        pairs = self.__dict__.setdefault("_slot_pairs", {})
        if C not in pairs:
            n = ops.BN_SLOTS * 2 * C
            pairs[C] = [torch.zeros(n, device=self.device), torch.zeros(n, device=self.device), -1]
        pair = pairs[C]
        use = 0 if pair[2] != 0 else 1
        pair[2] = use
        return pair[use], pair[use ^ 1]

    def reset_slot_pairs(self):
        pairs = self.__dict__.get("_slot_pairs", {})
        if not pairs:
            return
        if self.__dict__.get("_slot_arena_pairs") != len(pairs):
            arena = torch.zeros(sum(2 * p[0].numel() for p in pairs.values()), device=self.device)
            off = 0
            for p in pairs.values():
                n = p[0].numel()
                p[0], p[1], p[2] = arena[off:off + n], arena[off + n:off + 2 * n], -1
                off += 2 * n
            self._slot_arena, self._slot_arena_pairs = arena, len(pairs)
            return
        if any(p[2] >= 0 for p in pairs.values()):
            self._slot_arena.zero_()
            for p in pairs.values():
                p[2] = -1

    def partials(self, out):
        B, Hp, Wp, C = out.shape
        need = ((B * (Hp - 2) * (Wp - 2) + 255) // 256) * 2 * C
        if getattr(self, "_partials", None) is None or self._partials.numel() < need:
            self._partials = torch.empty(need, device=self.device)
        return self._partials

    def buf(self, key, B, H, W, C):
        k = (key, B, H, W, C)
        if k not in self._bufs:
            self._bufs[k] = ops.padded(B, H, W, C, self.device, self.act_dtype)
        return self._bufs[k]

    def conv(self, name, cin, cout, k, stride, init="kaiming_a0"):
        c = Conv(self.store, name, cin, cout, k, stride, self.gen, init)
        if self._side is not None:
            c.side_stream = self._side
        self.convs.append(c)
        return c

    def set_reference_fp32(self, on=True):
        self.join_side_stream()
        self.act_dtype = torch.float32 if on else torch.bfloat16
        self.fuse_eval = not on
        self._bufs = {}
        self._seg_ops = {}
        self.__dict__.pop("_seg_skip", None)
        for c in self.convs:
            c._plans = {}
        self._share_calibrated = True
        self.refresh_derived_weights()

    def set_overlap(self, on):
        self.join_side_stream()
        for c in self.convs + list(getattr(self, "dws", [])):
            c.side_stream = self._side if on else None
        self._overlap = bool(on)

    def set_cu_share(self, gbps_per_cu=47.0, target_us=200.0, min_cus=16, max_cus=128, join=False, calibrate=True,
                     split_reduce=True, split_target_us=190.0):
        self.join_side_stream()
        self.cu_share_report = None
        self._share_join = bool(join)
        self._share_split = bool(split_reduce), float(split_target_us)
        if gbps_per_cu is not None and not ops.cu_topology_is_mi355x(self.device):
            self._cu_share = None
            self._share_calibrated = True
            self.cu_share_report = {"enabled": False, "reason": "not a 256-CU / 8-XCD device: the CU split is MI355X's"}
            return
        self._cu_share = None if gbps_per_cu is None else (float(gbps_per_cu), float(target_us),
                                                           max(8, int(min_cus)), int(max_cus))
        self._share_calibrated = not calibrate

    def _split_us(self, grid_pixels, B):
        return self.share_stage_us.get(grid_pixels, self._share_split[1]) * (B / 512.0 if self.share_scale_batch else 1.0)

    def _share_plan(self, conv, x, elements, tensors, us=None):
        gbps, us0, lo, hi = self._cu_share
        B, Hp, Wp, _ = x.shape
        desc = conv.plan(B, Hp - 2, Wp - 2)[3]
        budget, n = ops.plan_cu_share(desc, elements, tensors, gbps, us0 if us is None else us, lo, hi)
        return desc, budget, n

    def _share_pair(self, conv, x, gout, elements, tensors, us=None):
        _, budget, n = self._share_plan(conv, x, elements, tensors, us)
        conv.backward_weight(x, gout, cu_budget=budget)
        return n

    def _calibration_unit(self):
        return None

    def calibrate_cu_share(self, comm=None):
        self._share_calibrated = True
        if self._cu_share is None:
            return self.cu_share_report
        if ops.is_deterministic():
            self.cu_share_report = {"enabled": True, "decided_by": "deterministic mode (schedule pinned, not timed)"}
            return self.cu_share_report
        if torch.cuda.is_current_stream_capturing():
            raise RuntimeError("calibrate_cu_share() synchronises with the host: call it (or run one eager step) "
                               "before capturing the step in a hipGraph")
        u = self._calibration_unit()
        if u is None or self._side is None or getattr(self, "_B", None) is None:
            self._cu_share = None
            self.cu_share_report = {"enabled": False, "reason": "no unit / second stream / forward to calibrate on"}
            return self.cu_share_report
# ... 107 lines not shown
            frows, drows, off, tf, td = [], [], 0, 0, 0

            def ntile(r):
                r32 = r // 32
                return 5 if r32 % 5 == 0 else 4 if r32 % 4 == 0 else 2 if r32 % 2 == 0 else 1

            wd_off = {}
            o = 0
            for c in self.convs:
                wd_off[c.name] = o
                o += c.numel()
            for c in dense:
                frows.append([self.store.entries[c.name][0], off, c.cout, c.cin, tf])
                drows.append([wd_off[c.name], off, c.cin, c.cout, td])
                c.wt_fwd = self._wt_fwd[off:off + c.numel()]
                c.wt_dgrad = self._wt_dgrad[off:off + c.numel()]
                off += c.numel()
                tf += (c.cout // (32 * ntile(c.cout))) * (c.cin // 32) * 9
                td += (c.cin // (32 * ntile(c.cin))) * (c.cout // 32) * 9
            self._wt_ftable = torch.tensor(frows, dtype=torch.int64, device=self.device)
            self._wt_dtable = torch.tensor(drows, dtype=torch.int64, device=self.device)
            self._wt_ftotal, self._wt_dtotal = tf, td
        self.refresh_derived_weights()

    def refresh_derived_weights(self):
        for b in self.bns:
            b._affine = None
        if self.act_dtype == torch.float32:
            for c in self.convs:
                c.wd32 = self.store.p(c.name).flip(1).permute(2, 1, 0).contiguous()
        if self._wt_n:
            ops.weight_tile_batched(self.store.bf16, self._wt_ftable, self._wt_n, self._wt_ftotal, self._wt_fwd)
        self._retile_seg(False)
        if self._side is None or not getattr(self, "_overlap", True):
            ops.weight_prep_batched(self.store.flat, self._wd_table, len(self.convs), self._wd_total, self._wd_flat)
            if self._wt_n:
                ops.weight_tile_batched(self._wd_flat, self._wt_dtable, self._wt_n, self._wt_dtotal, self._wt_dgrad)
            self._retile_seg(True)
            return
        self._side.wait_stream(torch.cuda.current_stream(self.device))
        with torch.cuda.stream(self._side):
            ops.weight_prep_batched(self.store.flat, self._wd_table, len(self.convs), self._wd_total, self._wd_flat)
            if self._wt_n:
                ops.weight_tile_batched(self._wd_flat, self._wt_dtable, self._wt_n, self._wt_dtotal, self._wt_dgrad)
            self._retile_seg(True)

    def sgd_step(self, lr, momentum=0.9, weight_decay=5e-4, grad_scale=1.0, zero_grad=False):
        self.join_side_stream()
        s = self.store
        ops.sgd_step(s.flat, s.grad, s.mom, lr, momentum, weight_decay, grad_scale, s.bf16, zero_grad=zero_grad)
        self._grad_is_zero = bool(zero_grad)
        self.refresh_derived_weights()

    def zero_grad(self):
        if not getattr(self, "_grad_is_zero", False):
            self.store.zero_grad()
        self._grad_is_zero = False

    def extra_param_views(self, buf):
        return {}

    def named_params(self, which="flat"):
        buf = {"flat": self.store.flat, "grad": self.store.grad, "bf16": self.store.bf16}[which]
        out = dict(self.extra_param_views(buf))
        for c in self.convs:
            out[c.name] = c.logical(buf)
        for b in self.bns:
            out[b.name + ".weight"] = self.store._view(buf, b.name + ".weight")[:b.c_real]
            out[b.name + ".bias"] = self.store._view(buf, b.name + ".bias")[:b.c_real]
        return out

    def named_buffers(self):
        out = {}
        for b in self.bns:
            out[b.name + ".running_mean"] = b.running_mean[:b.c_real]
            out[b.name + ".running_var"] = b.running_var[:b.c_real]
            out[b.name + ".num_batches_tracked"] = torch.tensor(b.num_batches_tracked, dtype=torch.long)
        return out

    def load_state_dict(self, sd):
        params, bufs = self.named_params("flat"), self.named_buffers()
        missing = {m for m in (set(params) | set(bufs)) - set(sd) if not m.endswith("num_batches_tracked")}
        if missing:
            raise KeyError(f"state dict is missing {sorted(missing)[:5]} ...")
        for name, view in list(params.items()) + list(bufs.items()):
            if name in sd and not name.endswith("num_batches_tracked"):
                view.copy_(sd[name].to(self.device))
        for b in self.bns:
            if b.name + ".num_batches_tracked" in sd:
                b.num_batches_tracked = int(sd[b.name + ".num_batches_tracked"])
        self.store.refresh_bf16()
        self.refresh_derived_weights()

    def state_dict(self):
        out = {k: v.detach().clone().contiguous() for k, v in self.named_params("flat").items()}
        out.update({k: v.detach().clone() for k, v in self.named_buffers().items()})
        return out

    def _tensor(self, key, shape):
        k = (key,) + tuple(shape)
        if k not in self._bufs:
            self._bufs[k] = torch.empty(shape, dtype=torch.float32, device=self.device)
        return self._bufs[k]

    def _zeroed(self, key, shape):
        k = (key, "zeroed") + tuple(shape)
        if k not in self._bufs:
            self._bufs[k] = torch.zeros(shape, dtype=torch.float32, device=self.device)
        return self._bufs[k]


class WRNEngine(_Engine):

    def __init__(self, num_classes=10, blocks=28, width_factor=10, in_size=(32, 32), device="cuda", seed=0):
        super().__init__(device, seed)
        assert (blocks - 4) % 6 == 0
        self.num_classes = num_classes
        self.in_size = in_size
        layers = [(blocks - 4) // 6] * 3
        widths = [16 * width_factor, 32 * width_factor, 64 * width_factor]
        self.stem_c = 16
        self.stem_cpad = _pad32(16)
        gen = self.gen
        bound = math.sqrt(2.0) * math.sqrt(3.0 / 27)
        self.store.add("features.init_block.weight", (self.stem_c, 3, 3, 3),
                       lambda v: v.uniform_(-bound, bound, generator=gen))
        self.units = []
        cin = 16
        for i, (n, cout) in enumerate(zip(layers, widths)):
            for j in range(n):
                stride = 2 if (j == 0 and i != 0) else 1
                pre = f"features.stage{i + 1}.unit{j + 1}."
                u = {
                    "bn1": self.bn(pre + "body.conv1.bn", cin),
                    "conv1": self.conv(pre + "body.conv1.conv.weight", cin, cout, 3, stride),
                    "bn2": self.bn(pre + "body.conv2.bn", cout),
                    "conv2": self.conv(pre + "body.conv2.conv.weight", cout, cout, 3, 1),
                    "idconv": (self.conv(pre + "identity_conv.weight", cin, cout, 1, stride)
                               if (cin != cout or stride != 1) else None),
                    "cin": cin, "cout": cout, "stride": stride, "key": f"s{i + 1}u{j + 1}",
                }
                self.units.append(u)
                cin = cout
        self.feat_c = cin
        self.post_bn = self.bn("features.post_activ.bn", cin)
        kb = 1.0 / math.sqrt(cin)
        self.store.add("output.weight", (num_classes, cin), lambda v: v.uniform_(-kb, kb, generator=gen))
        self.store.add("output.bias", (num_classes,), lambda v: v.uniform_(-kb, kb, generator=gen))
        self.finalize()
        self._img = None
        self._side = side_stream(self.device)
        for c in self.convs:
            c.side_stream = self._side
        self.set_cu_share(47.0)
        self.share_stage_us = {1024: 190.0, 256: 170.0}

    def _seg_conv1(self, u, B, h, w):
        c = u["conv1"]
        return self.seg_op((u["key"], "conv1", B, h, w), lambda: ops.seg_fwd_s2(B, h, w, c.cin, c.cout),
                           lambda: [self.store.pb(c.name).view(c.cout, 9 * c.cin)],
                           lambda: [self.store.p(c.name).view(c.cout, 9 * c.cin)])

    def _seg_conv2_sc(self, u, B, ho, wo):
        c2, ci = u["conv2"], u["idconv"]
        key = (u["key"], "conv2sc", B, ho, wo)
        if key in self._seg_ops:
            return self._seg_ops[key]
        skip = self.__dict__.setdefault("_seg_skip", set())
        if key in skip:
            return None
        try:
            plan = ops.seg_conv3x3_plus_1x1(B, ho, wo, c2.cin, c2.cout, ci.cin, (4 if u["stride"] == 2 else 1) * ci.cin)
        except _C.NBDTHipError:
            plan = None
        if plan is None or (plan.tile != 512 and not getattr(self, "seg_fuse_half_tiles", False)):
            skip.add(key)
            return None
        return self.seg_op(key, lambda: plan,
                           lambda: [self.store.pb(c2.name).view(c2.cout, 9 * c2.cin), self.store.pb(ci.name).view(ci.cout, ci.cin)],
                           lambda: [self.store.p(c2.name).view(c2.cout, 9 * c2.cin), self.store.p(ci.name).view(ci.cout, ci.cin)])

    def _seg_dgrad(self, u, B, hi, wi):
        c1, ci = u["conv1"], u["idconv"]
        if u["stride"] == 2:
            build = lambda: ops.seg_dgrad_s2(B, hi, wi, c1.cin, c1.cout, shortcut=True)
        else:
            build = lambda: ops.seg_dgrad3x3_plus_1x1(B, hi, wi, c1.cin, c1.cout)
        return self.seg_op((u["key"], "dgrad", B, hi, wi), build,
                           lambda: [c1.wd.view(c1.cin, 9 * c1.cout), ci.wd.view(ci.cin, ci.cout)],
                           lambda: [c1.wd32.view(c1.cin, 9 * c1.cout), ci.wd32.view(ci.cin, ci.cout)], on_side=True)

    def _calibration_unit(self):
        for u in self.units:
            if u["idconv"] is None and u["cout"] == self.units[0]["cout"]:
                return u
        return None

    classifier_names = ("output.weight", "output.bias")

    def forward(self, img, training=None, head=True):
        training = self.training if training is None else training
        if img.dtype != torch.float32 or not img.is_contiguous():
            img = img.float().contiguous()
        B, _, H, W = img.shape
        self._img, self._B = img, B
        x = self.buf("x0", B, H, W, self.stem_cpad)
        ops.stem_conv(img, self.store.p("features.init_block.weight"), x, self.stem_c)
        h, w = H, W
        x_has_stats = False
        for u in self.units:
            k, s = u["key"], u["stride"]
            cin, cout = _pad32(u["cin"]), _pad32(u["cout"])
            ho, wo = h // s, w // s
            t = self.buf(k + ".t", B, ho, wo, cout)
            a2 = self.buf(k + ".a2", B, ho, wo, cout)
            out = self.buf(k + ".out", B, ho, wo, cout)
            fuse = training and self.fuse_stats
            u["bn1"].stats(x, training, fused=fuse and x_has_stats)
            seg = training and self.use_seg and u["idconv"] is not None
            u["seg"] = seg
            if seg and s == 2:
                a1 = self.s2d_buf(k + ".a1", B, h, w, cin)
                ops.bn_apply_s2d(x, u["bn1"].mean, u["bn1"].rstd, u["bn1"].gamma, u["bn1"].beta, a1, relu=True)
            else:
                a1 = self.buf(k + ".a1", B, h, w, cin)
                u["bn1"].apply(x, a1, relu=True)
            if not training and self.fuse_eval:
                u["conv1"].forward_affine(a1, a2, u["bn2"], act=1)
            else:
                if seg and s == 2:
                    self._seg_conv1(u, B, h, w)([a1], t, bn_scratch=self.partials(t) if fuse else None)
                else:
                    u["conv1"].forward(a1, t, bn_scratch=self.partials(t) if fuse else None)
                u["bn2"].stats(t, training, fused=fuse)
                u["bn2"].apply(t, a2, relu=True)
            both = self._seg_conv2_sc(u, B, ho, wo) if seg else None
            if both is not None:
                both([a2, a1], out, bn_scratch=self.partials(out) if fuse else None)
            else:
                if u["idconv"] is not None:
                    idn = self.buf(f"idn{cout}", B, ho, wo, cout)
                    if seg and s == 2:
                        u["idconv"].forward_s2d(a1, idn, h, w)
                    else:
                        u["idconv"].forward(a1, idn)
                    res = idn
                else:
                    res = x
                u["conv2"].forward(a2, out, residual=res, bn_scratch=self.partials(out) if fuse else None)
            x_has_stats = True
            u["x_in"], u["x_out"] = x, out
            x, h, w = out, ho, wo
        self._x_last, self._hw = x, (h, w)
        self.post_bn.stats(x, training, fused=training and self.fuse_stats)
        self._pooled = self._tensor("pooled", (B, self.feat_c))
        ops.bn_relu_pool(x, self.post_bn.mean, self.post_bn.rstd, self.post_bn.gamma, self.post_bn.beta,
                         self._pooled)
        if not head:
            return self._pooled
        z = self._tensor("z", (B, self.num_classes))
        ops.linear_fwd(self._pooled, self.store.p("output.weight"), self.store.p("output.bias"), z)
        return z

    def grad_buckets(self):
        ent = self.store.entries
        s2 = ent["features.stage2.unit1.body.conv1.bn.weight"][0]
        s3 = ent["features.stage3.unit1.body.conv1.bn.weight"][0]
        return [(s3, self.store.grad.numel()), (s2, s3), (0, s2)]

    def backward(self, gz, comm=None, gpooled=None):
        self._grad_is_zero = False
        B = self._B
        self.join_side_stream()
        if self._cu_share is not None and not self._share_calibrated:
            self.calibrate_cu_share(comm)
        self.reset_slot_pairs()
        two_streams = self._side is not None and self._overlap
        buckets = self.grad_buckets() if comm is not None else None
        st = self.store
        if gpooled is not None:
            gpool = gpooled
        else:
            gz = gz.contiguous()
            gpool = self._tensor("gpool", (B, self.feat_c))
            ops.linear_bwd(self._pooled, st.p("output.weight"), gz, gpool, st.g("output.weight"), st.g("output.bias"))
        h, w = self._hw
        C = _pad32(self.feat_c)
        g = self.buf(f"g_out{C}", B, h, w, C)
        pb = self.post_bn
        ops.pool_bn_bwd(gpool, self._x_last, pb.mean, pb.rstd, pb.gamma, pb.beta, self.scratch(C), pb.dsum,
                        st.g(pb.name + ".weight"), st.g(pb.name + ".bias"), g)
        toggle, n_unit, side_mark = 0, 0, None
        if two_streams:
            self._side.wait_stream(torch.cuda.current_stream(self.device))
        for u in reversed(self.units):
            if two_streams and self.debug_join_each_unit:
                self.join_side_stream()
            elif two_streams:
                main = torch.cuda.current_stream(self.device)
                if side_mark is not None:
                    main.wait_event(side_mark)
                side_mark = torch.cuda.Event()
                side_mark.record(self._side)
            k, s = u["key"], u["stride"]
            cin, cout = _pad32(u["cin"]), _pad32(u["cout"])
            ho, wo = h, w
            hi, wi = ho * s, wo * s
            seg = bool(u.get("seg"))
            a1 = self.s2d_buf(k + ".a1", B, hi, wi, cin) if (seg and s == 2) else self.buf(k + ".a1", B, hi, wi, cin)
            t = self.buf(k + ".t", B, ho, wo, cout)
            a2 = self.buf(k + ".a2", B, ho, wo, cout)
            tag = ("@" + k) if self.debug_keep else ""
            ga2 = self.buf(f"ga2_{cout}{tag}", B, ho, wo, cout)
            gt = self.buf(f"gt_{cout}_{n_unit & 1}{tag}", B, ho, wo, cout)
            ga1 = self.buf(f"ga1_{cin}_{hi}{tag}", B, hi, wi, cin)
            toggle = (toggle + 1) % 3
            n_unit += 1
            g_in = self.buf(f"g_in{cin}_{hi}_{toggle}{tag}", B, hi, wi, cin)
            u["dbg"] = {"g_out": g, "ga2": ga2, "gt": gt, "ga1": ga1, "g_in": g_in}
            fuse = self.fuse_stats
            share = self._cu_share is not None and fuse and (two_streams or self.debug_share_serial)
            split = share and self._share_split[0]
            fused_here = bool(split and self.share_fused_hw and ho * wo >= self.share_fused_hw and not seg)
            if fused_here:
                split = False
            split_us = self._split_us(ho * wo, B)
            if self._cu_share is not None and self._share_split[0] and fuse and not share:
                fuse = False
            if split:
                u["conv2"].backward_data(g, ga2)
                n2 = self._share_pair(u["conv2"], a2, g, B * ho * wo * cout, self.share_bn2_tensors, split_us)
                u["bn2"].backward_cus(ga2, t, gt, n2)
                if self._share_join:
                    self.join_side_stream()
            elif fuse:
                if not share:
                    u["conv2"].backward_weight(a2, g)
                u["conv2"].backward_data(g, ga2, bn=u["bn2"], bn_x=t, partials=self.partials(t))
                n2 = self._share_pair(u["conv2"], a2, g, B * ho * wo * cout, 3,
                                      self.share_fused_target_us if fused_here else None) if share else 0
                u["bn2"].backward_fused(ga2, t, gt, self.partials(t), cus=n2)
                if share and self._share_join:
                    self.join_side_stream()
            else:
                u["conv2"].backward_weight(a2, g)
                u["conv2"].backward_data(g, ga2)
                u["bn2"].backward(ga2, None, t, gt, relu=True)
            if split and u["idconv"] is None:
                x_in = u["x_in"]
                u["conv1"].backward_data(gt, ga1)
                n1 = self._share_pair(u["conv1"], a1, gt, B * hi * wi * cin, self.share_bn1_tensors, split_us)
                u["bn1"].backward_cus(ga1, x_in, g_in, n1, gx_add=g)
                g, h, w = g_in, hi, wi
                continue
            if fuse and u["idconv"] is None:
                x_in = u["x_in"]
                if not share:
                    u["conv1"].backward_weight(a1, gt)
                u["conv1"].backward_data(gt, ga1, bn=u["bn1"], bn_x=x_in, partials=self.partials(x_in))
                n1 = self._share_pair(u["conv1"], a1, gt, B * hi * wi * cin, 4,
                                      self.share_fused_target_us if fused_here else None) if share else 0
                u["bn1"].backward_fused(ga1, x_in, g_in, self.partials(x_in), gx_add=g, cus=n1)
                g, h, w = g_in, hi, wi
                continue
            if seg:
                x_in = u["x_in"]
                if split and self.seg_share and (s == 2 or self.seg_share == "all"):
                    if self.seg_join == "all" or (self.seg_join == "small" and ho * wo <= 64):
                        self.join_side_stream()
                    self._seg_dgrad(u, B, hi, wi)([gt, g], ga1)
                    desc = u["conv1"].s2d_plan(B, hi, wi)[1] if s == 2 else u["conv1"].plan(B, hi, wi)[3]
                    gbps, _, lo, hi_cus = self._cu_share
                    budget, n1 = ops.plan_cu_share(desc, B * hi * wi * cin, self.share_bn2_tensors, gbps, split_us, lo, hi_cus)
                    if s == 2:
                        u["conv1"].backward_weight_s2d(a1, gt, hi, wi, cu_budget=budget)
                        u["idconv"].backward_weight_s2d(a1, g, hi, wi)
                    else:
                        u["conv1"].backward_weight(a1, gt, cu_budget=budget)
                        u["idconv"].backward_weight(a1, g)
                    u["bn1"].backward_cus(ga1, x_in, g_in, n1)
                else:
                    if s == 2:
                        u["conv1"].backward_weight_s2d(a1, gt, hi, wi)
                        u["idconv"].backward_weight_s2d(a1, g, hi, wi)
                    else:
                        u["conv1"].backward_weight(a1, gt)
                        u["idconv"].backward_weight(a1, g)
                    self._seg_dgrad(u, B, hi, wi)([gt, g], ga1)
                    u["bn1"].backward(ga1, None, x_in, g_in, relu=True)
                g, h, w = g_in, hi, wi
                if comm is not None and u["key"] in ("s3u1", "s2u1"):
                    self.join_side_stream()
                    comm.reduce_range(st.grad, *buckets[0 if u["key"] == "s3u1" else 1])
                    self._reserve_for(comm)
                continue
            u["conv1"].backward_weight(a1, gt)
            u["conv1"].backward_data(gt, ga1)
            if u["idconv"] is not None:
                u["idconv"].backward_weight(a1, g)
                u["idconv"].backward_data(g, ga1, accumulate=True)
                u["bn1"].backward(ga1, None, u["x_in"], g_in, relu=True)
            else:
                u["bn1"].backward(ga1, None, u["x_in"], g_in, relu=True, gx_add=g)
            g, h, w = g_in, hi, wi
            if comm is not None and u["key"] in ("s3u1", "s2u1"):
                self.join_side_stream()
                comm.reduce_range(st.grad, *buckets[0 if u["key"] == "s3u1" else 1])
                self._reserve_for(comm)
        ops.stem_wgrad(self._img, g, st.g("features.init_block.weight"), self.stem_c)
        self.join_side_stream()
        if comm is not None:
            comm.reduce_range(st.grad, *buckets[2])
            comm.finish(st.grad)
            self._reserve_for(None)

    def extra_param_views(self, buf):
        return {
            "features.init_block.weight": self.store._view(buf, "features.init_block.weight").permute(0, 3, 1, 2),
            "output.weight": self.store._view(buf, "output.weight"),
            "output.bias": self.store._view(buf, "output.bias"),
        }


class ResNetEngine(_Engine):

    def __init__(self, num_classes=10, num_blocks=(2, 2, 2, 2), device="cuda", seed=0):
        super().__init__(device, seed)
        self.num_classes = num_classes
        gen = self.gen
        self.stem_c = 64
        b0 = 1.0 / math.sqrt(27)
        self.store.add("conv1.weight", (64, 3, 3, 3), lambda v: v.uniform_(-b0, b0, generator=gen))
        self.bn0 = self.bn("bn1", 64)
        self.blocks = []
        cin = 64
        for i, (cout, stride0, n) in enumerate(zip((64, 128, 256, 512), (1, 2, 2, 2), num_blocks)):
            for j in range(n):
                stride = stride0 if j == 0 else 1
                pre = f"layer{i + 1}.{j}."
                short = stride != 1 or cin != cout
                blk = {
                    "conv1": self.conv(pre + "conv1.weight", cin, cout, 3, stride, init="torch_default"),
                    "bn1": self.bn(pre + "bn1", cout),
                    "conv2": self.conv(pre + "conv2.weight", cout, cout, 3, 1, init="torch_default"),
                    "bn2": self.bn(pre + "bn2", cout),
                    "sconv": self.conv(pre + "shortcut.0.weight", cin, cout, 1, stride, init="torch_default") if short else None,
                    "sbn": self.bn(pre + "shortcut.1", cout) if short else None,
                    "cin": cin, "cout": cout, "stride": stride, "key": f"l{i + 1}b{j}",
                }
                self.blocks.append(blk)
                cin = cout
        self.feat_c = cin
        kb = 1.0 / math.sqrt(cin)
        self.store.add("linear.weight", (num_classes, cin), lambda v: v.uniform_(-kb, kb, generator=gen))
        self.store.add("linear.bias", (num_classes,), lambda v: v.uniform_(-kb, kb, generator=gen))
        self.finalize()
        self._side = side_stream(self.device)
        for c in self.convs:
            c.side_stream = self._side
        self.res_share = (47.0, 15.0, 16, 128)
        dev = self.device
        self._id_mean = torch.zeros(cin, device=dev)
        self._id_rstd = torch.ones(cin, device=dev)
        self._id_gamma = torch.ones(cin, device=dev)
        self._id_beta = torch.zeros(cin, device=dev)
        self._id_dsum = torch.zeros(2 * cin, device=dev)

    def extra_param_views(self, buf):
        return {
            "conv1.weight": self.store._view(buf, "conv1.weight").permute(0, 3, 1, 2),
            "linear.weight": self.store._view(buf, "linear.weight"),
            "linear.bias": self.store._view(buf, "linear.bias"),
        }

    def grad_buckets(self):
        ent = self.store.entries
        l3 = ent["layer3.0.conv1.weight"][0]
        l2 = ent["layer2.0.conv1.weight"][0]
        return [(l3, self.store.grad.numel()), (l2, l3), (0, l2)]

    classifier_names = ("linear.weight", "linear.bias")

    def forward(self, img, training=None, head=True):
        training = self.training if training is None else training
        if img.dtype != torch.float32 or not img.is_contiguous():
            img = img.float().contiguous()
        B, _, H, W = img.shape
        self._img, self._B = img, B
        t0 = self.buf("t0", B, H, W, 64)
        x = self.buf("a0", B, H, W, 64)
        ops.stem_conv(img, self.store.p("conv1.weight"), t0, 64)
        self.bn0.stats(t0, training)
        self.bn0.apply(t0, x, relu=True)
        h, w = H, W
        for blk in self.blocks:
            k, s, cin, cout = blk["key"], blk["stride"], blk["cin"], blk["cout"]
            ho, wo = h // s, w // s
            a1 = self.buf(k + ".a1", B, ho, wo, cout)
            out = self.buf(k + ".out", B, ho, wo, cout)
            fuse = training and self.fuse_stats
            if not training and self.fuse_eval:
                blk["conv1"].forward_affine(x, a1, blk["bn1"], act=1)
                if blk["sconv"] is not None:
                    sc = self.buf(f"sc{cout}", B, ho, wo, cout)
                    blk["sconv"].forward_affine(x, sc, blk["sbn"], act=0)
                    res = sc
                else:
                    res = x
                blk["conv2"].forward_affine(a1, out, blk["bn2"], act=1, residual=res)
                blk["x_in"] = x
                x, h, w = out, ho, wo
                continue
            t1 = self.buf(k + ".t1", B, ho, wo, cout)
            t2 = self.buf(k + ".t2", B, ho, wo, cout)
            scr = self.partials(t1) if fuse else None
            blk["conv1"].forward(x, t1, bn_scratch=scr)
            blk["bn1"].stats(t1, training, fused=fuse)
            blk["bn1"].apply(t1, a1, relu=True)
            blk["conv2"].forward(a1, t2, bn_scratch=scr)
            blk["bn2"].stats(t2, training, fused=fuse)
            if blk["sconv"] is not None:
                ts = self.buf(k + ".ts", B, ho, wo, cout)
                sc = self.buf(f"sc{cout}", B, ho, wo, cout)
                blk["sconv"].forward(x, ts, bn_scratch=scr)
                blk["sbn"].stats(ts, training, fused=fuse)
                blk["sbn"].apply(ts, sc, relu=False)
                res = sc
            else:
                res = x
            blk["bn2"].apply(t2, out, relu=True, residual=res)
            blk["x_in"] = x
            x, h, w = out, ho, wo
        self._x_last, self._hw = x, (h, w)
        self._pooled = self._tensor("pooled", (B, self.feat_c))
        ops.bn_relu_pool(x, self._id_mean, self._id_rstd, self._id_gamma, self._id_beta, self._pooled)
# ... 172 lines not shown
```

neural-backed-decision-trees_amd/nbdt/ops.py:

```python
import ctypes

import torch

from nbdt import _C
from nbdt._C import ConvDesc, WgradDesc, check, lib, ptr

BN_SLOTS = 32
BN_EPS = 1e-5
BN_MOMENTUM = 0.1


def set_deterministic(on):
    check(lib().nbdt_set_deterministic(1 if on else 0))


def is_deterministic():
    return bool(lib().nbdt_get_deterministic())


def set_wgrad_store_epilogue(on):
    check(lib().nbdt_set_wgrad_store_epilogue(1 if on else 0))


def wgrad_store_epilogue():
# ... 150 lines not shown
        d.tap_off[0] = 0
        d.w_tap[0] = 0
        d.x_base = rowi + cin
    d.x_bs, d.x_hs, d.x_ws = (Hi + 2) * rowi, stride * rowi, stride * cin
    rowo = (Wo + 2) * cout
    d.g_bs, d.g_hs, d.g_ws, d.g_base = (Ho + 2) * rowo, rowo, cout, rowo + cout
    return d



class KernelTimer:

    def __init__(self, only=None):
        self.items = []
        self.only = only
        self.kernels = {}

    def wants(self, kind):
        return self.only is None or kind in self.only

    def bracket(self, kind, flops, device):
        s = torch.cuda.Event(enable_timing=True)
        e = torch.cuda.Event(enable_timing=True)
        self.items.append((kind, flops, s, e))
        return s, e

    def count(self, kernel_name):
        self.kernels[kernel_name] = self.kernels.get(kernel_name, 0) + 1

    def summary(self):
        torch.cuda.synchronize()
        out = {}
        for kind, flops, s, e in self.items:
            d = out.setdefault(kind, {"launches": 0, "flops": 0.0, "ms": 0.0})
            d["launches"] += 1
            d["flops"] += flops
            d["ms"] += s.elapsed_time(e)
        for d in out.values():
            d["avg_us"] = 1e3 * d["ms"] / max(d["launches"], 1)
            d["tflops"] = d["flops"] / (d["ms"] * 1e-3) / 1e12 if d["ms"] > 0 else 0.0
        return out


_timer = None


def set_timer(t):
    global _timer
    _timer = t



def conv_igemm(desc, inp, w_bf16, out, residual=None, bn_scratch=None):
    if _ref(inp):
        check(lib().nbdt_ref_conv(ctypes.byref(desc), ptr(inp), ptr(w_bf16), ptr(out), ptr(residual),
                                  stream_ptr(inp.device)))
        if bn_scratch is not None:
            B, H, W, C = _dims(out)
            check(lib().nbdt_ref_bn_stats(ptr(out), B, H, W, C, BN_EPS, BN_MOMENTUM, None, None, None, None,
                                          ptr(bn_scratch), stream_ptr(inp.device)))
        return
    ev = None
    if _timer is not None and _timer.wants("conv_igemm"):
        flops = desc_flops(desc)
        ev = _timer.bracket("conv_igemm", flops, inp.device)
        ev[0].record()
    if bn_scratch is None:
        check(lib().nbdt_conv_igemm(ctypes.byref(desc), ptr(inp), ptr(w_bf16), ptr(out), ptr(residual),
                                    stream_ptr(inp.device)))
    else:
        check(lib().nbdt_conv_igemm_stats(ctypes.byref(desc), ptr(inp), ptr(w_bf16), ptr(out), ptr(residual),
                                          ptr(bn_scratch), stream_ptr(inp.device)))
    if ev is not None:
        ev[1].record()
        _timer.count(last_igemm_kernel_full())


def desc_flops(desc):
    cin, cout = getattr(desc, "flop_channels", (desc.cin, desc.cout))
    return 2.0 * desc.B * desc.gh * desc.gw * desc.ntaps * cin * cout


def conv_igemm_multi(descs, inp, w_bf16, out):
    if _ref(inp):
        for d in descs:
            check(lib().nbdt_ref_conv(ctypes.byref(d), ptr(inp), ptr(w_bf16), ptr(out), None, stream_ptr(inp.device)))
        return
    arr = (ConvDesc * len(descs))(*descs)
    ev = None
    if _timer is not None and _timer.wants("conv_igemm"):
        flops = sum(desc_flops(d) for d in descs)
        ev = _timer.bracket("conv_igemm", flops, inp.device)
        ev[0].record()
    check(lib().nbdt_conv_igemm_multi(arr, len(descs), ptr(inp), ptr(w_bf16), ptr(out), stream_ptr(inp.device)))
    if ev is not None:
        ev[1].record()
        _timer.count(last_igemm_kernel_full())


def conv_igemm_bnbwd(desc, inp, w_bf16, out, bn_x, mean, rstd, gamma, beta, partials):
    _no_ref(inp, "conv_igemm_bnbwd (fused BatchNorm-backward sums): use the split or the unfused schedule")
    ev = None
    if _timer is not None and _timer.wants("conv_igemm"):
        flops = desc_flops(desc)
        ev = _timer.bracket("conv_igemm", flops, inp.device)
        ev[0].record()
    check(lib().nbdt_conv_igemm_bnbwd(ctypes.byref(desc), ptr(inp), ptr(w_bf16), ptr(out), ptr(bn_x), ptr(mean),
                                      ptr(rstd), ptr(gamma), ptr(beta), ptr(partials), stream_ptr(inp.device)))
    if ev is not None:
        ev[1].record()
        _timer.count(last_igemm_kernel_full())


def conv_igemm_affine(desc, inp, w_bf16, out, scale, shift, act=1, residual=None):
    _no_ref(inp, "conv_igemm_affine (folded eval-mode BatchNorm): engine.fuse_eval is off in reference mode")
    check(lib().nbdt_conv_igemm_affine(ctypes.byref(desc), ptr(inp), ptr(w_bf16), ptr(out), ptr(residual),
                                       ptr(scale), ptr(shift), act, stream_ptr(inp.device)))


def bn_bwd_fused(gy, x, mean, rstd, gamma, beta, partials, dsum, dgamma, dbeta, gx, gx_add=None, cus=0):
    _no_ref(x, "bn_bwd_fused: use the split or the unfused schedule")
    B, H, W, C = _dims(x)
    st = stream_ptr(x.device)
    check(lib().nbdt_bn_bwd_fold(B, H, W, C, ptr(partials), ptr(dsum), ptr(dgamma), ptr(dbeta), st))
    if cus > 0:
        check(lib().nbdt_bn_bwd_apply_cus(ptr(gy), ptr(x), ptr(mean), ptr(rstd), ptr(gamma), ptr(beta), ptr(dsum),
                                          ptr(gx_add), B, H, W, C, ptr(gx), int(cus), st))
        return
    check(lib().nbdt_bn_bwd_apply(ptr(gy), None, ptr(x), ptr(mean), ptr(rstd), ptr(gamma), ptr(beta),
                                  ptr(dsum), ptr(gx_add), 1, B, H, W, C, ptr(gx), None, st))


def bn_bwd_cus(gy, x, mean, rstd, gamma, beta, scratch, dsum, dgamma, dbeta, gx, cus, gx_add=None):
    B, H, W, C = _dims(x)
    st = stream_ptr(x.device)
    if _ref(x):
        check(lib().nbdt_ref_bn_bwd(ptr(gy), None, None, ptr(x), ptr(mean), ptr(rstd), ptr(gamma), ptr(beta), 1,
                                    ptr(gx_add), B, H, W, C, 1, ptr(dsum), ptr(dgamma), ptr(dbeta), ptr(gx), None, st))
        return
    if isinstance(scratch, (tuple, list)):
        slots, other = scratch
        check(lib().nbdt_bn_bwd_cus(ptr(gy), ptr(x), ptr(mean), ptr(rstd), ptr(gamma), ptr(beta), ptr(gx_add), B, H, W,
                                    C, ptr(slots), ptr(other), ptr(dsum), ptr(dgamma), ptr(dbeta), ptr(gx), int(cus),
                                    st))
        return
    check(lib().nbdt_bn_bwd_reduce_cus(ptr(gy), ptr(x), ptr(mean), ptr(rstd), ptr(gamma), ptr(beta), B, H, W, C,
                                       ptr(scratch), ptr(dsum), ptr(dgamma), ptr(dbeta), int(cus), st))
    check(lib().nbdt_bn_bwd_apply_cus(ptr(gy), ptr(x), ptr(mean), ptr(rstd), ptr(gamma), ptr(beta), ptr(dsum),
                                      ptr(gx_add), B, H, W, C, ptr(gx), int(cus), st))


def conv_wgrad(desc, x, gy, dw, cu_budget=0):
    desc.cu_budget = int(cu_budget)
    if _ref(x):
        check(lib().nbdt_ref_wgrad(ctypes.byref(desc), ptr(x), ptr(gy), ptr(dw), stream_ptr(x.device)))
        return
    ev = None
    if _timer is not None and _timer.wants("conv_wgrad"):
        flops = desc_flops(desc)
        ev = _timer.bracket("conv_wgrad", flops, x.device)
        ev[0].record()
    check(lib().nbdt_conv_wgrad(ctypes.byref(desc), ptr(x), ptr(gy), ptr(dw), stream_ptr(x.device)))
    if ev is not None:
        ev[1].record()


def conv_wgrad_blocks(desc, cu_budget=0):
    desc.cu_budget = int(cu_budget)
    return int(lib().nbdt_conv_wgrad_blocks(ctypes.byref(desc)))


MI355X_CUS, MI355X_XCDS = 256, 8


def cu_topology_is_mi355x(device):
    props = torch.cuda.get_device_properties(device)
    return props.multi_processor_count == MI355X_CUS and "gfx950" in getattr(props, "gcnArchName", "gfx950")


def plan_cu_share(desc, elements, tensors, gbps_per_cu, target_us, min_cus, max_cus):
    held = (reserved_cus() + MI355X_XCDS - 1) // MI355X_XCDS
    per_xcd = MI355X_CUS // MI355X_XCDS - held
    cus = per_xcd * MI355X_XCDS
    n = int(round(elements * 2 * tensors / (gbps_per_cu * 1e9 * target_us * 1e-6)))
    n = max(max(8, int(min_cus)), min(int(max_cus), n))
    n = min(n, cus - MI355X_XCDS)
    while True:
        blocks = conv_wgrad_blocks(desc, cus - n)
        if not 0 < blocks <= cus - n:
            return cus - n, n
        free = MI355X_XCDS * (per_xcd - (blocks + MI355X_XCDS - 1) // MI355X_XCDS)
        if free >= MI355X_XCDS or n + MI355X_XCDS > cus - MI355X_XCDS:
            return cus - n, max(free, MI355X_XCDS)
        n += MI355X_XCDS


def weight_prep(w_fp32, cout, taps, cin, w_bf16=None, wd_bf16=None):
    check(lib().nbdt_weight_prep(ptr(w_fp32), cout, taps, cin, ptr(w_bf16), ptr(wd_bf16),
                                 stream_ptr(w_fp32.device)))


def weight_tile_batched(src_bf16, table, n, total, dst_bf16):
    check(lib().nbdt_weight_tile_batched(ptr(src_bf16), ptr(table), n, total, ptr(dst_bf16),
                                         stream_ptr(src_bf16.device)))


def weight_tiles(w_bf16):
    rows, taps, k = w_bf16.shape
    assert taps == 9 and rows % 32 == 0 and k % 32 == 0
    r32 = rows // 32
    nt = 5 if r32 % 5 == 0 else 4 if r32 % 4 == 0 else 2 if r32 % 2 == 0 else 1
    total = (rows // (32 * nt)) * (k // 32) * 9
    table = torch.tensor([[0, 0, rows, k, 0]], dtype=torch.int64, device=w_bf16.device)
    dst = torch.empty(rows * 9 * k, dtype=torch.bfloat16, device=w_bf16.device)
    weight_tile_batched(w_bf16.contiguous(), table, 1, total, dst)
    return dst


def last_igemm_kernel():
    return lib().nbdt_debug_last_igemm().decode()


def last_igemm_kernel_full():
    return lib().nbdt_debug_last_igemm_full().decode()


def last_wgrad_kernel():
    return lib().nbdt_debug_last_wgrad().decode()


def weight_prep_batched(flat, table, n_layers, total, wd_flat):
    check(lib().nbdt_weight_prep_batched(ptr(flat), ptr(table), n_layers, total, ptr(wd_flat),
                                         stream_ptr(flat.device)))


def _dims(t):
    B, Hp, Wp, C = t.shape
    return B, Hp - 2, Wp - 2, C


def bn_stats(x, scratch, save_mean, save_rstd, running_mean=None, running_var=None,
             eps=BN_EPS, momentum=BN_MOMENTUM, slots_filled=False):
    B, H, W, C = _dims(x)
    if _ref(x):
        check(lib().nbdt_ref_bn_stats(ptr(x), B, H, W, C, eps, momentum, ptr(running_mean), ptr(running_var),
                                      ptr(save_mean), ptr(save_rstd), None, stream_ptr(x.device)))
        return
    check(lib().nbdt_bn_stats(None if slots_filled else ptr(x), B, H, W, C, eps, momentum, ptr(running_mean), ptr(running_var),
                              ptr(scratch), ptr(save_mean), ptr(save_rstd), stream_ptr(x.device)))


def bn_finalize(x, scratch, save_mean, save_rstd, running_mean=None, running_var=None,
                eps=BN_EPS, momentum=BN_MOMENTUM):
    B, H, W, C = _dims(x)
    check(lib().nbdt_bn_finalize(B, H, W, C, eps, momentum, ptr(running_mean), ptr(running_var), ptr(scratch),
                                 ptr(save_mean), ptr(save_rstd), stream_ptr(x.device)))


def bn_apply(x, mean, rstd, gamma, beta, y, relu=True, residual=None):
    B, H, W, C = _dims(x)
    if _ref(x):
        check(lib().nbdt_ref_bn_apply(ptr(x), ptr(mean), ptr(rstd), ptr(gamma), ptr(beta), ptr(residual),
                                      1 if relu else 0, B, H, W, C, ptr(y), stream_ptr(x.device)))
        return
    check(lib().nbdt_bn_apply(ptr(x), ptr(mean), ptr(rstd), ptr(gamma), ptr(beta), ptr(residual),
                              1 if relu else 0, B, H, W, C, ptr(y), stream_ptr(x.device)))


def bn_bwd(gy, y, x, mean, rstd, gamma, scratch, dsum, dgamma, dbeta, gx, relu=True, gx_add=None,
           g_resid=None, beta=None):
    B, H, W, C = _dims(x)
    st = stream_ptr(x.device)
    r = 1 if relu else 0
    if _ref(x):
        check(lib().nbdt_ref_bn_bwd(ptr(gy), None, ptr(y), ptr(x), ptr(mean), ptr(rstd), ptr(gamma), ptr(beta), r,
                                    ptr(gx_add), B, H, W, C, 1, ptr(dsum), ptr(dgamma), ptr(dbeta), ptr(gx), ptr(g_resid),
                                    st))
        return
    check(lib().nbdt_bn_bwd_reduce(ptr(gy), ptr(y), ptr(x), ptr(mean), ptr(rstd), ptr(gamma), ptr(beta), r,
                                   B, H, W, C, ptr(scratch), ptr(dsum), ptr(dgamma), ptr(dbeta), st))
    check(lib().nbdt_bn_bwd_apply(ptr(gy), ptr(y), ptr(x), ptr(mean), ptr(rstd), ptr(gamma), ptr(beta),
                                  ptr(dsum), ptr(gx_add), r, B, H, W, C, ptr(gx), ptr(g_resid), st))


def bn_relu_pool(x, mean, rstd, gamma, beta, pooled):
    B, H, W, C = _dims(x)
    if _ref(x):
        check(lib().nbdt_ref_bn_relu_pool(ptr(x), ptr(mean), ptr(rstd), ptr(gamma), ptr(beta), B, H, W, C, ptr(pooled),
                                          stream_ptr(x.device)))
        return
    check(lib().nbdt_bn_relu_pool(ptr(x), ptr(mean), ptr(rstd), ptr(gamma), ptr(beta), B, H, W, C,
                                  ptr(pooled), stream_ptr(x.device)))


def pool_bn_bwd(gpooled, x, mean, rstd, gamma, beta, scratch, dsum, dgamma, dbeta, gx):
    B, H, W, C = _dims(x)
    st = stream_ptr(x.device)
    if _ref(x):
        check(lib().nbdt_ref_bn_bwd(None, ptr(gpooled), None, ptr(x), ptr(mean), ptr(rstd), ptr(gamma), ptr(beta), 1,
                                    None, B, H, W, C, 1, ptr(dsum), ptr(dgamma), ptr(dbeta), ptr(gx), None, st))
        return
    check(lib().nbdt_pool_bn_bwd_reduce(ptr(gpooled), ptr(x), ptr(mean), ptr(rstd), ptr(gamma), ptr(beta),
                                        B, H, W, C, ptr(scratch), ptr(dsum), ptr(dgamma), ptr(dbeta), st))
    check(lib().nbdt_pool_bn_bwd_apply(ptr(gpooled), ptr(x), ptr(mean), ptr(rstd), ptr(gamma), ptr(beta),
                                       ptr(dsum), B, H, W, C, ptr(gx), st))


def pool_bn_bwd_apply(gpooled, x, mean, rstd, gamma, beta, dsum, gx):
    B, H, W, C = _dims(x)
    st = stream_ptr(x.device)
    if _ref(x):
        check(lib().nbdt_ref_bn_bwd(None, ptr(gpooled), None, ptr(x), ptr(mean), ptr(rstd), ptr(gamma), ptr(beta), 1,
                                    None, B, H, W, C, 0, ptr(dsum), None, None, ptr(gx), None, st))
        return
    check(lib().nbdt_pool_bn_bwd_apply(ptr(gpooled), ptr(x), ptr(mean), ptr(rstd), ptr(gamma), ptr(beta), ptr(dsum),
                                       B, H, W, C, ptr(gx), st))


def stem_conv(img, w, out, cout_real, stride=1):
    B, _, H, W = img.shape
    if _ref(out):
        check(lib().nbdt_ref_stem_conv(ptr(img), ptr(w), B, H, W, cout_real, out.shape[3], stride, ptr(out),
                                       stream_ptr(img.device)))
        return
    check(lib().nbdt_stem_conv(ptr(img), ptr(w), B, H, W, cout_real, out.shape[3], stride, ptr(out),
                               stream_ptr(img.device)))


def stem_wgrad(img, gy, dw, cout_real, stride=1):
    B, _, H, W = img.shape
    if _ref(gy):
        check(lib().nbdt_ref_stem_wgrad(ptr(img), ptr(gy), B, H, W, cout_real, gy.shape[3], stride, ptr(dw),
                                        stream_ptr(img.device)))
        return
    check(lib().nbdt_stem_wgrad(ptr(img), ptr(gy), B, H, W, cout_real, gy.shape[3], stride, ptr(dw),
                                stream_ptr(img.device)))


def linear_fwd(x, w, b, z):
    B, K = x.shape
    N = w.shape[0]
# ... 339 lines not shown
```

Measured before the change: 32120 images/sec.

## Fuse stride-2 conv1 and 1x1 shortcut weight-gradient into one s2d pair launch

Adds a paired space-to-depth weight-gradient launch that computes both the 3x3 stride-2 conv1 weight gradient and the 1x1 shortcut (idconv) weight gradient in a single kernel grid. Shortcut work items are appended after the conv1 items and reuse the same input activation tiles. This removes a separate kernel launch and a second pass over the activations, and lets both jobs share the CU budget. It is enabled by default in the CU-share path and adds a new shortcut device function with its own LDS pipeline and split planning, which could change occupancy or load balance.

```diff
diff --git a/include/nbdt_hip.h b/include/nbdt_hip.h
--- a/include/nbdt_hip.h
+++ b/include/nbdt_hip.h
@@ -144,6 +144,9 @@
 int nbdt_conv_wgrad(const nbdt_wgrad_desc* d, const void* x, const void* gy, float* dw,
                     void* stream);
 int nbdt_conv_wgrad_blocks(const nbdt_wgrad_desc* d);
+int nbdt_conv_wgrad_s2d_pair(const nbdt_wgrad_desc* d, const void* x, const void* gy, float* dw, const void* gy_sc,
+                             float* dw_sc, void* stream);
+int nbdt_conv_wgrad_s2d_pair_blocks(const nbdt_wgrad_desc* d);
 
 int nbdt_weight_prep(const float* w, int32_t cout, int32_t taps, int32_t cin, void* w_bf16,
                      void* wd_bf16, void* stream);
diff --git a/neural-backed-decision-trees_amd/csrc/common.h b/neural-backed-decision-trees_amd/csrc/common.h
--- a/neural-backed-decision-trees_amd/csrc/common.h
+++ b/neural-backed-decision-trees_amd/csrc/common.h
@@ -143,8 +143,9 @@
 int wgrad_taps_blocks(const nbdt_wgrad_desc* d);
 
 bool wgrad_s2d_applicable(const nbdt_wgrad_desc* d);
-int wgrad_s2d(const nbdt_wgrad_desc* d, const void* x, const void* gy, float* dw, hipStream_t st);
-int wgrad_s2d_blocks(const nbdt_wgrad_desc* d);
+int wgrad_s2d(const nbdt_wgrad_desc* d, const void* x, const void* gy, float* dw, const void* gsc, float* dwsc,
+              hipStream_t st);
+int wgrad_s2d_blocks(const nbdt_wgrad_desc* d, bool pair);
 
 struct BnBwdArgs {
   const void* x;
diff --git a/neural-backed-decision-trees_amd/csrc/rules.hip b/neural-backed-decision-trees_amd/csrc/rules.hip
--- a/neural-backed-decision-trees_amd/csrc/rules.hip
+++ b/neural-backed-decision-trees_amd/csrc/rules.hip
@@ -999,7 +999,7 @@
 
 
 extern "C" const char* nbdt_last_error(void) { return nbdt::g_err; }
-extern "C" int nbdt_version(void) { return 108; }
+extern "C" int nbdt_version(void) { return 109; }
 extern "C" int nbdt_device_count(void) {
   int n = 0;
   if (hipGetDeviceCount(&n) != hipSuccess) return 0;
diff --git a/neural-backed-decision-trees_amd/csrc/wgrad.hip b/neural-backed-decision-trees_amd/csrc/wgrad.hip
--- a/neural-backed-decision-trees_amd/csrc/wgrad.hip
+++ b/neural-backed-decision-trees_amd/csrc/wgrad.hip
@@ -19,7 +19,8 @@
   const int64_t M_all = (int64_t)d->B * d->gh * d->gw;
   NBDT_REQUIRE(M_all < (1ll << 31), "pixel grid too large");
   if (nbdt::wgrad_taps_applicable(d)) return nbdt::wgrad_taps(d, x, gy, dw, (hipStream_t)stream);
-  if (d->variant != 3 && nbdt::wgrad_s2d_applicable(d)) return nbdt::wgrad_s2d(d, x, gy, dw, (hipStream_t)stream);
+  if (d->variant != 3 && nbdt::wgrad_s2d_applicable(d))
+    return nbdt::wgrad_s2d(d, x, gy, dw, nullptr, nullptr, (hipStream_t)stream);
   NBDT_REQUIRE(d->variant == 0 || d->variant == 3, "variant 2 / 4 / 5 select between the dense 3x3 stride-1 kernels only");
   nbdt::g_last_wgrad = "conv_wgrad_dma_kernel";
   return nbdt::wgrad_dma(d, x, gy, dw, (hipStream_t)stream);
@@ -29,8 +30,36 @@
   if (!d || d->cin <= 0 || d->cin % 32 != 0 || d->cout <= 0 || d->cout % 32 != 0 || d->ntaps != 9) return 0;
   if (d->B <= 0 || d->gh <= 0 || d->gw <= 0) return 0;
   if (d->cu_budget != 0 && (d->cu_budget < 32 || d->cu_budget > 256)) return 0;
-  if (d->variant != 3 && nbdt::wgrad_s2d_applicable(d)) return nbdt::wgrad_s2d_blocks(d);
+  if (d->variant != 3 && nbdt::wgrad_s2d_applicable(d)) return nbdt::wgrad_s2d_blocks(d, false);
   return nbdt::wgrad_taps_blocks(d);
+}
+
+static int s2d_pair_check(const nbdt_wgrad_desc* d) {
+  NBDT_REQUIRE(d->cin > 0 && d->cin % 32 == 0 && d->cout > 0 && d->cout % 32 == 0, "channels must be multiples of 32");
+  NBDT_REQUIRE(d->B > 0 && d->gh > 0 && d->gw > 0, "empty pixel grid");
+  NBDT_REQUIRE(d->g_bs % 8 == 0 && d->g_base % 8 == 0, "pixel offsets must be 16-byte aligned");
+  NBDT_REQUIRE(d->cu_budget == 0 || (d->cu_budget >= 32 && d->cu_budget <= 256), "cu_budget must be 0 or 32..256");
+  NBDT_REQUIRE(d->variant == 0, "the pair launch has no variants");
+  NBDT_REQUIRE((int64_t)d->B * d->gh * d->gw < (1ll << 31), "pixel grid too large");
+  NBDT_REQUIRE(nbdt::wgrad_s2d_applicable(d), "not a space-to-depth 3x3 stride-2 weight-gradient descriptor");
+  return NBDT_OK;
+}
+
+extern "C" int nbdt_conv_wgrad_s2d_pair(const nbdt_wgrad_desc* d, const void* x, const void* gy, float* dw,
+                                        const void* gy_sc, float* dw_sc, void* stream) {
+  NBDT_REQUIRE(d && x && gy_sc && dw_sc, "null argument");
+  NBDT_REQUIRE((gy == nullptr) == (dw == nullptr), "gy and dw are both given or both null");
+  const int rc = s2d_pair_check(d);
+  if (rc != NBDT_OK) return rc;
+  return nbdt::wgrad_s2d(d, x, gy, dw, gy_sc, dw_sc, (hipStream_t)stream);
+}
+
+extern "C" int nbdt_conv_wgrad_s2d_pair_blocks(const nbdt_wgrad_desc* d) {
+  if (!d || d->cin <= 0 || d->cin % 32 != 0 || d->cout <= 0 || d->cout % 32 != 0 || d->variant != 0) return 0;
+  if (d->B <= 0 || d->gh <= 0 || d->gw <= 0) return 0;
+  if (d->cu_budget != 0 && (d->cu_budget < 32 || d->cu_budget > 256)) return 0;
+  if (!nbdt::wgrad_s2d_applicable(d)) return 0;
+  return nbdt::wgrad_s2d_blocks(d, true);
 }
 
 namespace nbdt { thread_local const char* g_last_wgrad = ""; }
diff --git a/neural-backed-decision-trees_amd/csrc/wgrad_s2d.hip b/neural-backed-decision-trees_amd/csrc/wgrad_s2d.hip
--- a/neural-backed-decision-trees_amd/csrc/wgrad_s2d.hip
+++ b/neural-backed-decision-trees_amd/csrc/wgrad_s2d.hip
@@ -23,7 +23,243 @@
   int stages_per_row, rowgroups;
   int x_pix;
   FastDiv div_spr, div_rg;
+  int items1;
+  int sc_nb, sc_groups;
+  const bf16_t* gsc;
+  float* dwsc;
+  long long dwsc_split_stride;
 };
+}
+
+template <int WM>
+__device__ __forceinline__ void s2d_shortcut_item(const nbdt::WgradS2dParams& p, int item) {
+  constexpr int CG = 32 * WM;
+  constexpr int KSP = 64;
+  constexpr int PG = 2 * CG;
+  constexpr int G_BYTES = KSP * PG;
+  constexpr int G_INSTR = G_BYTES / 1024;
+  constexpr int IPG = (G_INSTR + 7) / 8;
+  constexpr int IPX = 3;
+  constexpr int NSLOT = 4, PD = 3;
+  constexpr int NB = 5;
+  extern __shared__ __attribute__((aligned(16))) unsigned char smem[];
+
+  const nbdt_wgrad_desc& d = p.d;
+  const int tid = threadIdx.x;
+  const int lane = tid & 63;
+  const int wave = __builtin_amdgcn_readfirstlane(tid >> 6);
+  const int grp = wave >> 2, w4 = wave & 3;
+  const int wm = w4 >> 1, wn = w4 & 1;
+
+#define NBDT_PIN(x) __builtin_amdgcn_readfirstlane(x)
+  const int nb = NBDT_PIN(p.sc_nb);
+  const int n_tiles = (d.cout / CG) * p.sc_groups;
+  const int tile = item % n_tiles;
+  const int split = item / n_tiles;
+  const int co_blk = tile / p.sc_groups;
+  const int co0 = co_blk * CG;
+  const int ci0 = (tile - co_blk * p.sc_groups) * 32 * nb;
+  const int s_begin = split * p.stages_per_split;
+  int s_end = s_begin + p.stages_per_split;
+  s_end = s_end < p.stages ? s_end : p.stages;
+  if (s_begin >= s_end) return;
+  const int n_st = s_end - s_begin;
+
+  const int g_hs = NBDT_PIN(d.g_hs), g_ws = NBDT_PIN(d.g_ws), g_bs = NBDT_PIN(d.g_bs);
+  const int x_bs = NBDT_PIN(d.x_bs), x_hs = NBDT_PIN(d.x_hs), x_ws = NBDT_PIN(d.x_ws);
+  const int rs = NBDT_PIN(p.rs), cs = NBDT_PIN(p.cs);
+  const int x_instr = 4 * nb;
+  const int stage_bytes = G_BYTES + x_instr * 1024;
+  FastDiv dspr, drg;
+  dspr.mul = NBDT_PIN(p.div_spr.mul); dspr.sh = NBDT_PIN(p.div_spr.sh); dspr.d = NBDT_PIN(p.div_spr.d);
+  drg.mul = NBDT_PIN(p.div_rg.mul); drg.sh = NBDT_PIN(p.div_rg.sh); drg.d = NBDT_PIN(p.div_rg.d);
+  const unsigned long long gy_u = (unsigned long long)p.gsc, x_u = (unsigned long long)p.x;
+  const bf16_t* gy_base = (const bf16_t*)(((unsigned long long)NBDT_PIN((unsigned)(gy_u >> 32)) << 32) |
+                                          (unsigned)NBDT_PIN((unsigned)gy_u));
+  const bf16_t* x_base = (const bf16_t*)(((unsigned long long)NBDT_PIN((unsigned)(x_u >> 32)) << 32) |
+                                         (unsigned)NBDT_PIN((unsigned)x_u));
+#undef NBDT_PIN
+
+  const unsigned lds_base = (unsigned)(size_t)(__attribute__((address_space(3))) unsigned char*)smem;
+  unsigned g_voff[IPG];
+#pragma unroll
+  for (int k = 0; k < IPG; ++k) {
+    const int pos = (wave + 8 * k) * 1024 + lane * 16;
+    int px = pos / PG;
+    const int j = (pos - px * PG) >> 4;
+    const int src_chunk = j ^ (((px >> 3) & 1) << 1);
+    px = px < KSP ? px : KSP - 1;
+    g_voff[k] = (unsigned)((px / cs) * g_hs + (px % cs) * g_ws + d.g_base + co0 + src_chunk * 8) * 2u;
+  }
+  unsigned x_voff[IPX];
+#pragma unroll
+  for (int k = 0; k < IPX; ++k) {
+    int slot = 16 * (wave + 8 * k) + (lane >> 2);
+    slot = slot < 64 * nb ? slot : 64 * nb - 1;
+    const int b = slot >> 6, kk = slot & 63;
+    const int i = kk / cs, j = kk - i * cs;
+    const int src_chunk = (lane & 3) ^ ((((j >> 3) ^ i) & 1) << 1);
+    x_voff[k] = (unsigned)((i + 1) * x_hs + (j + 1) * x_ws + ci0 + 32 * b + src_chunk * 8) * 2u;
+  }
+  int n_mine = 0;
+#pragma unroll
+  for (int k = 0; k < IPX; ++k) n_mine += (wave + 8 * k < x_instr) ? 1 : 0;
+#pragma unroll
+  for (int k = 0; k < IPG; ++k) n_mine += (wave + 8 * k < G_INSTR) ? 1 : 0;
+
+  auto stage_off = [&](int stage, int& g_stage, int& x_stage) {
+    const unsigned st = (unsigned)stage;
+    const unsigned q1m = __umulhi(st, dspr.mul) >> dspr.sh;
+    const unsigned q1 = dspr.d == 1 ? st : q1m;
+    const int sc = (int)(st - q1 * dspr.d);
+    const unsigned bm = __umulhi(q1, drg.mul) >> drg.sh;
+    const unsigned b = drg.d == 1 ? q1 : bm;
+    const int rg = (int)(q1 - b * drg.d);
+    const int r0 = rg * rs, c0 = sc * cs;
+    g_stage = (int)b * g_bs + r0 * g_hs + c0 * g_ws;
+    x_stage = (int)b * x_bs + r0 * x_hs + c0 * x_ws;
+  };
+  auto issue = [&](int slot_i, int g_stage, int x_stage) {
+    const unsigned dst0 = lds_base + slot_i * stage_bytes;
+#pragma unroll
+    for (int k = 0; k < IPG; ++k)
+      if (wave + 8 * k < G_INSTR) glds16_s(gy_base + g_stage, g_voff[k], dst0 + (wave + 8 * k) * 1024);
+#pragma unroll
+    for (int k = 0; k < IPX; ++k)
+      if (wave + 8 * k < x_instr) glds16_s(x_base + x_stage, x_voff[k], dst0 + G_BYTES + (wave + 8 * k) * 1024);
+  };
+
+  f32x4 acc[NB][WM];
+#pragma unroll
+  for (int b = 0; b < NB; ++b)
+#pragma unroll
+    for (int a = 0; a < WM; ++a) acc[b][a] = f32x4{0.f, 0.f, 0.f, 0.f};
+
+  typedef const __attribute__((address_space(3))) unsigned char* lds_cptr;
+  typedef __attribute__((address_space(3))) s16x4* lds_tr;
+  const lds_cptr smem3 = (lds_cptr)smem;
+  const int g4 = lane >> 4, t16 = lane & 15;
+  const int pr = t16 >> 2;
+  const int c8 = (t16 & 3) * 8;
+  lds_cptr ga[2];
+#pragma unroll
+  for (int a = 0; a < 2; ++a)
+    ga[a] = smem3 + (grp * 32 + 8 * g4 + pr) * PG + (((wm * WM + a) ^ (g4 & 1)) * 32) + c8;
+  lds_cptr xa;
+  {
+    const int k = grp * 32 + 8 * g4;
+    const int i = k / cs, j = k - i * cs + pr;
+    xa = smem3 + G_BYTES + c8 + (((i * cs + j) << 6) | (((((j >> 3) ^ i) ^ wn) & 1) << 5));
+  }
+
+#pragma unroll
+  for (int u = 0; u < PD; ++u)
+    if (u < n_st) {
+      int gs, xs;
+      stage_off(s_begin + u, gs, xs);
+      issue(u, gs, xs);
+    }
+  asm volatile("s_waitcnt vmcnt(0)" ::: "memory");
+  __builtin_amdgcn_s_barrier();
+  if (grp == 1) __builtin_amdgcn_s_barrier();
+  __builtin_amdgcn_sched_barrier(0);
+
+  auto advance = [&](int from_slot, int to_slot) {
+    int delta = (to_slot - from_slot) * stage_bytes;
+    asm volatile("" : "+s"(delta));
+    ga[0] += delta;
+    ga[1] += delta;
+    xa += delta;
+  };
+  int slot_c = 0, slot_n = 1 % NSLOT, slot_d = PD % NSLOT;
+  int g_next = 0, x_next = 0;
+  if (PD < n_st) stage_off(s_begin + PD, g_next, x_next);
+
+  for (int u = 0; u < n_st; ++u) {
+    bf16x8 gf[WM];
+    u32x2 xw[NB][2];
+#pragma unroll
+    for (int a = 0; a < WM; ++a) {
+      const lds_cptr a0 = ga[a & 1] + (a >> 1) * 64;
+      const s16x4 lo = __builtin_amdgcn_ds_read_tr16_b64_v4i16((lds_tr)(a0));
+      const s16x4 hi = __builtin_amdgcn_ds_read_tr16_b64_v4i16((lds_tr)(a0 + 4 * PG));
+      gf[a] = bf16x8{lo[0], lo[1], lo[2], lo[3], hi[0], hi[1], hi[2], hi[3]};
+    }
+#pragma unroll
+    for (int b = 0; b < NB; ++b)
+      if (b < nb) {
+        xw[b][0] = __builtin_bit_cast(u32x2, __builtin_amdgcn_ds_read_tr16_b64_v4i16((lds_tr)(xa + 4096 * b)));
+        xw[b][1] = __builtin_bit_cast(u32x2, __builtin_amdgcn_ds_read_tr16_b64_v4i16((lds_tr)(xa + 4096 * b + 256)));
+      }
+    if (u + PD <= n_st) {
+      switch (n_mine) {
+#define NBDT_CASE(K) case K: asm volatile("s_waitcnt vmcnt(%0)" ::"n"(K) : "memory"); break;
+        NBDT_CASE(1) NBDT_CASE(2) NBDT_CASE(3) NBDT_CASE(4) NBDT_CASE(5) NBDT_CASE(6)
+#undef NBDT_CASE
+        default: asm volatile("s_waitcnt vmcnt(0)" ::: "memory"); break;
+      }
+    } else {
+      asm volatile("s_waitcnt vmcnt(0)" ::: "memory");
+    }
+    if (u + PD < n_st) issue(slot_d, g_next, x_next);
+    asm volatile("s_waitcnt lgkmcnt(0)" ::: "memory");
+    __builtin_amdgcn_sched_barrier(0);
+    __builtin_amdgcn_s_barrier();
+    __builtin_amdgcn_sched_barrier(0);
+    __builtin_amdgcn_s_setprio(1);
+    advance(slot_c, slot_n);
+    stage_off(s_begin + u + 1 + PD, g_next, x_next);
+#pragma unroll
+    for (int b = 0; b < NB; ++b)
+      if (b < nb) {
+        const bf16x8 xf = __builtin_bit_cast(bf16x8, u32x4_t{xw[b][0][0], xw[b][0][1], xw[b][1][0], xw[b][1][1]});
+#pragma unroll
+        for (int a = 0; a < WM; ++a)
+          acc[b][a] = __builtin_amdgcn_mfma_f32_16x16x32_bf16(gf[a], xf, acc[b][a], 0, 0, 0);
+      }
+    asm volatile("" : "+v"(xa), "+v"(ga[0]), "+v"(ga[1]));
+    __builtin_amdgcn_s_setprio(0);
+    __builtin_amdgcn_sched_barrier(0);
+    __builtin_amdgcn_s_barrier();
+    __builtin_amdgcn_sched_barrier(0);
+    slot_c = slot_n;
+    slot_n = slot_n + 1 == NSLOT ? 0 : slot_n + 1;
+    slot_d = slot_d + 1 == NSLOT ? 0 : slot_d + 1;
+  }
+  if (grp == 0) __builtin_amdgcn_s_barrier();
+  __builtin_amdgcn_sched_barrier(0);
+  {
+    typedef __attribute__((address_space(3))) f32x4* lds_f4;
+    const lds_f4 ex = (lds_f4)(__attribute__((address_space(3))) unsigned char*)smem + (w4 * (NB * WM) * 64 + lane);
+    if (grp == 1) {
+#pragma unroll
+      for (int b = 0; b < NB; ++b)
+        if (b < nb)
+#pragma unroll
+          for (int a = 0; a < WM; ++a) ex[(b * WM + a) * 64] = acc[b][a];
+    }
+    __syncthreads();
+    if (grp == 1) return;
+#pragma unroll
+    for (int b = 0; b < NB; ++b)
+      if (b < nb)
+#pragma unroll
+        for (int a = 0; a < WM; ++a) acc[b][a] += ex[(b * WM + a) * 64];
+  }
+#pragma unroll
+  for (int b = 0; b < NB; ++b) {
+    if (b >= nb) continue;
+    const int ci = ci0 + 32 * b + wn * 16 + t16;
+#pragma unroll
+    for (int a = 0; a < WM; ++a)
+#pragma unroll
+      for (int r = 0; r < 4; ++r) {
+        const int co = co0 + (wm * WM + a) * 16 + 4 * g4 + r;
+        float* const dst = p.dwsc + (int64_t)split * p.dwsc_split_stride + (int64_t)co * d.cin + ci;
+        if (p.store) *dst = acc[b][a][r];
+        else atomicAdd(dst, acc[b][a][r]);
+      }
+  }
 }
 
 template <int WM>
@@ -47,7 +283,11 @@
 
   const int item = (blockIdx.x & 7) * p.per_xcd + (blockIdx.x >> 3);
   if (item >= p.items) return;
-  const int n_tiles = p.items / p.splits;
+  if (item >= p.items1) {
+    s2d_shortcut_item<WM>(p, item - p.items1);
+    return;
+  }
+  const int n_tiles = p.items1 / p.splits;
   const int tile = item % n_tiles;
   const int split = item / n_tiles;
   const int co_blk = tile / p.n_ci_blocks;
@@ -363,10 +603,13 @@
   return s2d_geometry(d, nullptr);
 }
 
-static void s2d_split(WgradS2dParams& p, int wm) {
+static void s2d_split(WgradS2dParams& p, int wm, bool conv1, int sc_nb) {
   const nbdt_wgrad_desc& d = p.d;
   p.n_ci_blocks = d.cin / 32;
-  const int tiles = (d.cout / (32 * wm)) * p.n_ci_blocks;
+  const int tiles1 = conv1 ? (d.cout / (32 * wm)) * p.n_ci_blocks : 0;
+  p.sc_nb = sc_nb;
+  p.sc_groups = sc_nb ? p.n_ci_blocks / sc_nb : 0;
+  const int tiles = tiles1 + (d.cout / (32 * wm)) * p.sc_groups;
   int cus = d.cu_budget > 0 ? d.cu_budget : 256;
   cus = std::max(8, std::min(cus, 256 - reserved_cus()));
   int splits = cus / tiles;
@@ -376,23 +619,35 @@
   p.stages_per_split = (p.stages + splits - 1) / splits;
   splits = (p.stages + p.stages_per_split - 1) / p.stages_per_split;
   p.splits = splits;
+  p.items1 = tiles1 * splits;
   p.items = tiles * splits;
   p.per_xcd = (p.items + 7) / 8;
 }
 
-int wgrad_s2d_blocks(const nbdt_wgrad_desc* d) {
+static int s2d_sc_nb(const nbdt_wgrad_desc* d) {
+  const int nci = d->cin / 32;
+  for (int nb = 5; nb >= 1; --nb)
+    if (nci % nb == 0 && 4 * ((size_t)64 * 64 * s2d_wm(d->cout) + (size_t)nb * 4096) <= 160 * 1024) return nb;
+  return 0;
+}
+
+int wgrad_s2d_blocks(const nbdt_wgrad_desc* d, bool pair) {
   WgradS2dParams p;
   p.d = *d;
   if (!s2d_geometry(d, &p)) return 0;
-  s2d_split(p, s2d_wm(d->cout));
+  const int sc_nb = pair ? s2d_sc_nb(d) : 0;
+  if (pair && !sc_nb) return 0;
+  s2d_split(p, s2d_wm(d->cout), true, sc_nb);
   return p.per_xcd * 8 < p.items ? p.per_xcd * 8 : p.items;
 }
 
 template <int WM>
-static int launch_s2d(WgradS2dParams& p, hipStream_t st) {
+static int launch_s2d(WgradS2dParams& p, hipStream_t st, bool conv1, int sc_nb) {
   const nbdt_wgrad_desc& d = p.d;
-  s2d_split(p, WM);
-  const size_t shmem = (size_t)4 * (64 * 64 * WM + (size_t)p.x_instr * 1024);
+  s2d_split(p, WM, conv1, sc_nb);
+  const size_t stage1 = (size_t)64 * 64 * WM + (size_t)p.x_instr * 1024;
+  const size_t stage_sc = (size_t)64 * 64 * WM + (size_t)sc_nb * 4096;
+  const size_t shmem = 4 * std::max(conv1 ? stage1 : 0, sc_nb ? stage_sc : 0);
   const void* fn = reinterpret_cast<const void*>(&conv_wgrad_s2d_kernel<WM>);
   static DeviceAttr site;
   if (site.need(shmem)) {
@@ -400,11 +655,14 @@
     site.done(shmem);
   }
   float* const dw = p.dw;
-  const size_t dw_elems = (size_t)d.cout * d.w_ntaps * d.cin;
+  float* const dwsc = p.dwsc;
+  const size_t dw_elems = conv1 ? (size_t)d.cout * d.w_ntaps * d.cin : 0;
+  const size_t sc_elems = sc_nb ? (size_t)d.cout * d.cin : 0;
   p.dw_split_stride = 0;
+  p.dwsc_split_stride = 0;
   p.store = ((wgrad_store_epilogue() && p.splits <= 64 && d.cu_budget == 0) || deterministic()) ? 1 : 0;
   if (p.store) {
-    float* rows = det_rows(st, (size_t)p.splits * dw_elems);
+    float* rows = det_rows(st, (size_t)p.splits * (dw_elems + sc_elems));
     if (!rows && !deterministic()) {
       p.store = 0;
     } else {
@@ -412,28 +670,42 @@
                                    nbdt::det_rows_why());
       p.dw = rows;
       p.dw_split_stride = (long long)dw_elems;
+      p.dwsc = rows + (size_t)p.splits * dw_elems;
+      p.dwsc_split_stride = (long long)sc_elems;
     }
   }
   void* args[] = {(void*)&p};
   NBDT_HIP_CHECK(hipLaunchKernel(fn, dim3(p.per_xcd * 8), dim3(512), args, shmem, st));
   g_last_wgrad = "conv_wgrad_s2d_kernel";
-  if (p.dw != dw) return det_fold(st, p.dw, p.splits, dw_elems, dw);
+  if (p.store) {
+    if (conv1) {
+      const int rc = det_fold(st, p.dw, p.splits, dw_elems, dw);
+      if (rc != NBDT_OK) return rc;
+    }
+    if (sc_nb) return det_fold(st, p.dwsc, p.splits, sc_elems, dwsc);
+  }
   return NBDT_OK;
 }
 
-int wgrad_s2d(const nbdt_wgrad_desc* d, const void* x, const void* gy, float* dw, hipStream_t st) {
+int wgrad_s2d(const nbdt_wgrad_desc* d, const void* x, const void* gy, float* dw, const void* gsc, float* dwsc,
+              hipStream_t st) {
   WgradS2dParams p;
   p.d = *d;
   p.x = (const bf16_t*)x;
   p.gy = (const bf16_t*)gy;
   p.dw = dw;
+  p.gsc = (const bf16_t*)gsc;
+  p.dwsc = dwsc;
   p.x_pix = 4 * d->cin;
   if (!s2d_geometry(d, &p)) return nbdt::fail(NBDT_EINVAL, "%s%s", "space-to-depth weight gradient: shape does not fit", "");
+  const bool conv1 = gy != nullptr;
+  const int sc_nb = gsc ? s2d_sc_nb(d) : 0;
+  if (gsc && !sc_nb) return nbdt::fail(NBDT_EINVAL, "%s%s", "space-to-depth weight gradient: the shortcut tile does not fit", "");
   const int wm = s2d_wm(d->cout);
-  if (wm == 5) return launch_s2d<5>(p, st);
-  if (wm == 4) return launch_s2d<4>(p, st);
-  if (wm == 2) return launch_s2d<2>(p, st);
-  return launch_s2d<1>(p, st);
-}
-
-}
+  if (wm == 5) return launch_s2d<5>(p, st, conv1, sc_nb);
+  if (wm == 4) return launch_s2d<4>(p, st, conv1, sc_nb);
+  if (wm == 2) return launch_s2d<2>(p, st, conv1, sc_nb);
+  return launch_s2d<1>(p, st, conv1, sc_nb);
+}
+
+}
diff --git a/neural-backed-decision-trees_amd/nbdt/_C.py b/neural-backed-decision-trees_amd/nbdt/_C.py
--- a/neural-backed-decision-trees_amd/nbdt/_C.py
+++ b/neural-backed-decision-trees_amd/nbdt/_C.py
@@ -86,6 +86,7 @@
     "nbdt_debug_last_igemm_full": (c_char_p, []),
     "nbdt_debug_last_wgrad": (c_char_p, []),
     "nbdt_conv_wgrad_blocks": (c_int, [_P]),
+    "nbdt_conv_wgrad_s2d_pair_blocks": (c_int, [_P]),
     "nbdt_conv_plan": (c_int, [_P, _P, _P]),
     "nbdt_soft_forward": (c_int, [c_void_p, _P, c_int, c_int64, c_int64, _P, _P]),
     "nbdt_soft_backward": (c_int, [c_void_p, _P, c_int, c_int64, c_int64, _P, _P, _P]),
@@ -119,6 +120,7 @@
     "nbdt_bn_bwd_cus": (c_int, [_P, _P, _P, _P, _P, _P, _P, c_int32, c_int32, c_int32, c_int32, _P, _P, _P, _P, _P, _P,
                                 c_int32, _P]),
     "nbdt_conv_wgrad": (c_int, [POINTER(WgradDesc), _P, _P, _P, _P]),
+    "nbdt_conv_wgrad_s2d_pair": (c_int, [POINTER(WgradDesc), _P, _P, _P, _P, _P, _P]),
     "nbdt_ref_conv": (c_int, [POINTER(ConvDesc), _P, _P, _P, _P, _P]),
     "nbdt_ref_wgrad": (c_int, [POINTER(WgradDesc), _P, _P, _P, _P]),
     "nbdt_ref_bn_stats": (c_int, [_P, c_int32, c_int32, c_int32, c_int32, c_float, c_float, _P, _P, _P, _P, _P, _P]),
diff --git a/neural-backed-decision-trees_amd/nbdt/engine.py b/neural-backed-decision-trees_amd/nbdt/engine.py
--- a/neural-backed-decision-trees_amd/nbdt/engine.py
+++ b/neural-backed-decision-trees_amd/nbdt/engine.py
@@ -192,6 +192,24 @@
         side.wait_stream(main)
         with torch.cuda.stream(side):
             ops.conv_wgrad(desc, xs, gout, self.store.g(self.name), cu_budget)
+
+    def s2d_pair_fits(self, B, Hi, Wi):
+        key = ("s2d_pair", B, Hi, Wi)
+        if key not in self._plans:
+            self._plans[key] = ops.conv_wgrad_s2d_pair_blocks(self.s2d_plan(B, Hi, Wi)[1]) > 0
+        return self._plans[key]
+
+    def backward_weight_s2d_pair(self, sc, xs, gout, gsc, Hi, Wi, cu_budget=0):
+        desc = self.s2d_plan(xs.shape[0], Hi, Wi)[1]
+        side = getattr(self, "side_stream", None)
+        args = (desc, xs, gout, self.store.g(self.name), gsc, sc.store.g(sc.name), cu_budget)
+        if side is None:
+            ops.conv_wgrad_s2d_pair(*args)
+            return
+        main = torch.cuda.current_stream(xs.device)
+        side.wait_stream(main)
+        with torch.cuda.stream(side):
+            ops.conv_wgrad_s2d_pair(*args)
 
     def backward_weight(self, x, gout, cu_budget=0):
         B, Hp, Wp, _ = x.shape
@@ -317,6 +335,7 @@
         self._seg_ops = {}
         self.seg_share = True
         self.seg_join = None
+        self.s2d_pair_wgrad = False
         self.share_fused_hw = 0
         self.share_stage_us = {}
         self.share_scale_batch = True
@@ -730,6 +749,7 @@
         self._side = side_stream(self.device)
         for c in self.convs:
             c.side_stream = self._side
+        self.s2d_pair_wgrad = True
         self.set_cu_share(47.0)
         self.share_stage_us = {1024: 190.0, 256: 170.0}
 
@@ -949,8 +969,12 @@
                     self._seg_dgrad(u, B, hi, wi)([gt, g], ga1)
                     desc = u["conv1"].s2d_plan(B, hi, wi)[1] if s == 2 else u["conv1"].plan(B, hi, wi)[3]
                     gbps, _, lo, hi_cus = self._cu_share
-                    budget, n1 = ops.plan_cu_share(desc, B * hi * wi * cin, self.share_bn2_tensors, gbps, split_us, lo, hi_cus)
-                    if s == 2:
+                    pair = s == 2 and self.s2d_pair_wgrad and u["conv1"].s2d_pair_fits(B, hi, wi)
+                    budget, n1 = ops.plan_cu_share(desc, B * hi * wi * cin, self.share_bn2_tensors, gbps, split_us, lo, hi_cus,
+                                                   s2d_pair=pair)
+                    if pair:
+                        u["conv1"].backward_weight_s2d_pair(u["idconv"], a1, gt, g, hi, wi, cu_budget=budget)
+                    elif s == 2:
                         u["conv1"].backward_weight_s2d(a1, gt, hi, wi, cu_budget=budget)
                         u["idconv"].backward_weight_s2d(a1, g, hi, wi)
                     else:
@@ -958,7 +982,9 @@
                         u["idconv"].backward_weight(a1, g)
                     u["bn1"].backward_cus(ga1, x_in, g_in, n1)
                 else:
-                    if s == 2:
+                    if s == 2 and self.s2d_pair_wgrad and u["conv1"].s2d_pair_fits(B, hi, wi):
+                        u["conv1"].backward_weight_s2d_pair(u["idconv"], a1, gt, g, hi, wi)
+                    elif s == 2:
                         u["conv1"].backward_weight_s2d(a1, gt, hi, wi)
                         u["idconv"].backward_weight_s2d(a1, g, hi, wi)
                     else:
diff --git a/neural-backed-decision-trees_amd/nbdt/ops.py b/neural-backed-decision-trees_amd/nbdt/ops.py
--- a/neural-backed-decision-trees_amd/nbdt/ops.py
+++ b/neural-backed-decision-trees_amd/nbdt/ops.py
@@ -326,17 +326,39 @@
 
 def conv_wgrad(desc, x, gy, dw, cu_budget=0):
     desc.cu_budget = int(cu_budget)
-    if _ref(x):
-        check(lib().nbdt_ref_wgrad(ctypes.byref(desc), ptr(x), ptr(gy), ptr(dw), stream_ptr(x.device)))
+    sc = getattr(desc, "s2d_shortcut", None)
+    if _ref(x):
+        if gy is not None:
+            check(lib().nbdt_ref_wgrad(ctypes.byref(desc), ptr(x), ptr(gy), ptr(dw), stream_ptr(x.device)))
+        if sc is not None:
+            d1 = conv_wgrad_desc_s2d(desc.B, 2 * desc.gh, 2 * desc.gw, desc.cin, desc.cout, 1)
+            check(lib().nbdt_ref_wgrad(ctypes.byref(d1), ptr(x), ptr(sc[0]), ptr(sc[1]), stream_ptr(x.device)))
         return
     ev = None
     if _timer is not None and _timer.wants("conv_wgrad"):
-        flops = desc_flops(desc)
+        taps = 9 if sc is None else (9 if gy is not None else 0) + 1
+        flops = desc_flops(desc) * taps / desc.ntaps
         ev = _timer.bracket("conv_wgrad", flops, x.device)
         ev[0].record()
-    check(lib().nbdt_conv_wgrad(ctypes.byref(desc), ptr(x), ptr(gy), ptr(dw), stream_ptr(x.device)))
+    if sc is None:
+        check(lib().nbdt_conv_wgrad(ctypes.byref(desc), ptr(x), ptr(gy), ptr(dw), stream_ptr(x.device)))
+    else:
+        check(lib().nbdt_conv_wgrad_s2d_pair(ctypes.byref(desc), ptr(x), ptr(gy), ptr(dw), ptr(sc[0]), ptr(sc[1]),
+                                             stream_ptr(x.device)))
     if ev is not None:
         ev[1].record()
+
+
+def s2d_pair_desc(desc, gy_sc, dw_sc):
+    d = WgradDesc.from_buffer_copy(desc)
+    if hasattr(desc, "flop_channels"):
+        d.flop_channels = desc.flop_channels
+    d.s2d_shortcut = (gy_sc, dw_sc)
+    return d
+
+
+def conv_wgrad_s2d_pair(desc, x, gy, dw, gy_sc, dw_sc, cu_budget=0):
+    conv_wgrad(s2d_pair_desc(desc, gy_sc, dw_sc), x, gy, dw, cu_budget)
 
 
 def conv_wgrad_blocks(desc, cu_budget=0):
@@ -344,6 +366,11 @@
     return int(lib().nbdt_conv_wgrad_blocks(ctypes.byref(desc)))
 
 
+def conv_wgrad_s2d_pair_blocks(desc, cu_budget=0):
+    desc.cu_budget = int(cu_budget)
+    return int(lib().nbdt_conv_wgrad_s2d_pair_blocks(ctypes.byref(desc)))
+
+
 MI355X_CUS, MI355X_XCDS = 256, 8
 
 
@@ -352,7 +379,7 @@
     return props.multi_processor_count == MI355X_CUS and "gfx950" in getattr(props, "gcnArchName", "gfx950")
 
 
-def plan_cu_share(desc, elements, tensors, gbps_per_cu, target_us, min_cus, max_cus):
+def plan_cu_share(desc, elements, tensors, gbps_per_cu, target_us, min_cus, max_cus, s2d_pair=False):
     held = (reserved_cus() + MI355X_XCDS - 1) // MI355X_XCDS
     per_xcd = MI355X_CUS // MI355X_XCDS - held
     cus = per_xcd * MI355X_XCDS
@@ -360,7 +387,7 @@
     n = max(max(8, int(min_cus)), min(int(max_cus), n))
     n = min(n, cus - MI355X_XCDS)
     while True:
-        blocks = conv_wgrad_blocks(desc, cus - n)
+        blocks = conv_wgrad_s2d_pair_blocks(desc, cus - n) if s2d_pair else conv_wgrad_blocks(desc, cus - n)
         if not 0 < blocks <= cus - n:
             return cus - n, n
         free = MI355X_XCDS * (per_xcd - (blocks + MI355X_XCDS - 1) // MI355X_XCDS)
```

Result: no change. 32350 images/sec (median of 6 runs) (+0.7%).
